# actionml/universal-recommender

Hardware: NVIDIA H100
Metric: CCO train events/sec to indicator model (higher is better)
Workload: dtype int32+f64

## Files before the change

universal_recommender_b200/csrc/cco_api.cu:

```cuda
#include <cuda_runtime.h>
#include <dlfcn.h>
#include <stdarg.h>
#include <stdio.h>
#include <stdlib.h>
#include <string.h>

#include <algorithm>
#include <charconv>
#include <cmath>
#include <functional>
#include <cub/cub.cuh>
#include <nvtx3/nvToolsExt.h>
#include <condition_variable>
#include <mutex>
#include <string>
#include <thread>
#include <unordered_map>
#include <vector>

#include "../../include/cco_b200.h"
#include "cco_kernels.cuh"
#include "cco_sampler.cuh"
#include "cco_format.cuh"
#include "cco_strings.cuh"
#include "cco_json.cuh"
#include "cco_events.cuh"
#include "cco_queries.cuh"
#include "cco_results.cuh"
#include "cco_index_pages.cuh"
#include "cco_index_write.cuh"
#include "cco_refresh.cuh"
#include "cco_intern.cuh"

namespace cco {

static thread_local char g_err[512] = "";
static int set_error(int code, const char *fmt, ...) {
  va_list ap;
  va_start(ap, fmt);
  vsnprintf(g_err, sizeof g_err, fmt, ap);
  va_end(ap);
  return code;
}
#define CK(expr)                                                                                      \
  do {                                                                                                \
    cudaError_t _e = (expr);                                                                          \
    if (_e != cudaSuccess)                                                                            \
      return set_error(_e == cudaErrorMemoryAllocation ? CCO_E_OOM : CCO_E_CUDA, "%s: %s (%s:%d)", #expr, \
                       cudaGetErrorString(_e), __FILE__, __LINE__);                                   \
  } while (0)
#define CKR(expr)            \
  do {                       \
    int _r = (expr);         \
    if (_r != CCO_OK) return _r; \
  } while (0)

typedef struct ncclComm *ncclComm_t;
typedef struct { char internal[128]; } ncclUniqueId;
struct Nccl {
  void *h = nullptr;
  int (*GetUniqueId)(ncclUniqueId *) = nullptr;
  int (*CommInitRank)(ncclComm_t *, int, ncclUniqueId, int) = nullptr;
  int (*CommInitAll)(ncclComm_t *, int, const int *) = nullptr;
  int (*CommDestroy)(ncclComm_t) = nullptr;
  int (*AllReduce)(const void *, void *, size_t, int, int, ncclComm_t, cudaStream_t) = nullptr;
  int (*AllGather)(const void *, void *, size_t, int, ncclComm_t, cudaStream_t) = nullptr;
  int (*Broadcast)(const void *, void *, size_t, int, int, ncclComm_t, cudaStream_t) = nullptr;
  int (*GroupStart)() = nullptr;
  int (*GroupEnd)() = nullptr;
  const char *(*GetErrorString)(int) = nullptr;
};
static Nccl g_nccl;
static std::mutex g_nccl_mu;
static int load_nccl() {
  std::lock_guard<std::mutex> lk(g_nccl_mu);
  if (g_nccl.h) return CCO_OK;
  void *h = dlopen("libnccl.so.2", RTLD_NOW | RTLD_GLOBAL);
  if (!h) h = dlopen("libnccl.so", RTLD_NOW | RTLD_GLOBAL);
  if (!h) return set_error(CCO_E_NCCL, "cannot load libnccl.so.2: %s", dlerror());
#define SYM(field, name)                                                         \
  *(void **)(&g_nccl.field) = dlsym(h, name);                                    \
  if (!g_nccl.field) return set_error(CCO_E_NCCL, "libnccl: missing symbol %s", name);
  SYM(GetUniqueId, "ncclGetUniqueId")
  SYM(CommInitRank, "ncclCommInitRank")
  SYM(CommInitAll, "ncclCommInitAll")
  SYM(CommDestroy, "ncclCommDestroy")
  SYM(AllReduce, "ncclAllReduce")
  SYM(AllGather, "ncclAllGather")
  SYM(Broadcast, "ncclBroadcast")
  SYM(GroupStart, "ncclGroupStart")
  SYM(GroupEnd, "ncclGroupEnd")
  SYM(GetErrorString, "ncclGetErrorString")
#undef SYM
  g_nccl.h = h;
  return CCO_OK;
}
constexpr int kNcclInt32 = 2, kNcclUint32 = 3, kNcclSum = 0, kNcclMax = 2;

}

using namespace cco;

struct PinnedBuf {
  void *p;
  size_t cap;
  bool used;
};

struct GroupShared {
  int world = 0;
  std::mutex mu;
  std::condition_variable cv;
  int arrived = 0;
  unsigned long long generation = 0;
  std::vector<long long> totals;
  struct cco_result *merged = nullptr;
  int status = 0;
  char err[512] = "";
  void barrier() {
    std::unique_lock<std::mutex> lk(mu);
    const unsigned long long g = generation;
    if (++arrived == world) {
      arrived = 0;
      ++generation;
      cv.notify_all();
    } else {
      cv.wait(lk, [&] { return generation != g; });
    }
  }
};

struct cco_ctx {
  int device = 0, rank = 0, world = 1;
  int sm_count = 0;
  size_t smem_optin = 0;
  cudaStream_t stream = nullptr, copy_stream = nullptr;
  cudaEvent_t ev[8] = {};
  cudaEvent_t tev[2] = {};
  cudaEvent_t copy_ev[2] = {};
  cudaStream_t bin_stream[8] = {};
  cudaStream_t sched_stream = nullptr;
  cudaEvent_t bin_ev[9] = {};
  std::vector<PinnedBuf> pinned;
  std::mutex mu;
  ncclComm_t comm = nullptr;
  int launches = 0;
  int32_t key_range_cap = 0;
  uint64_t intern_mask = ~0ULL;
  unsigned char *mail_h = nullptr, *mail_d = nullptr;
  size_t mail_used = 0;
  struct MailItem { void *dst; size_t off, n; int group; };
  std::vector<MailItem> mail_pending;
  std::vector<cudaEvent_t> mail_ev;
  int mail_group = 0;
  unsigned char *arena = nullptr;
  size_t arena_bytes = 0, arena_used = 0;
  int arena_live = 0;
  bool arena_registered = false;
  struct Slab { unsigned char *p; size_t cap; };
  std::vector<Slab> slabs;
  size_t slab_idx = 0, slab_off = 0;
  bool slab_busy = false;
  std::vector<cudaEvent_t> ev_timing, ev_plain;
  size_t ev_timing_used = 0, ev_plain_used = 0;
  std::vector<cco_ctx *> members;
  GroupShared *gshared = nullptr;

  void *pinned_get(size_t bytes, bool for_result = true) {
    std::lock_guard<std::mutex> lk(mu);
    if (bytes == 0) bytes = 16;
    if (arena && for_result) {
      const size_t off = (arena_used + 255) & ~(size_t)255;
      if (off + bytes <= arena_bytes) {
        arena_used = off + bytes;
        ++arena_live;
        return arena + off;
      }
    }
    int best = -1;
    for (size_t i = 0; i < pinned.size(); ++i)
      if (!pinned[i].used && pinned[i].cap >= bytes && (best < 0 || pinned[i].cap < pinned[best].cap)) best = (int)i;
    if (best >= 0) {
      pinned[best].used = true;
      return pinned[best].p;
    }
    void *p = nullptr;
    size_t cap = (bytes + (1u << 20) - 1) & ~((size_t)(1u << 20) - 1);
    if (cudaHostAlloc(&p, cap, cudaHostAllocPortable) != cudaSuccess) return nullptr;
    pinned.push_back({p, cap, true});
    return p;
  }
  void pinned_put(void *p) {
    std::lock_guard<std::mutex> lk(mu);
    if (arena && (unsigned char *)p >= arena && (unsigned char *)p < arena + arena_bytes) {
      if (--arena_live <= 0) { arena_live = 0; arena_used = 0; }
      return;
    }
    for (auto &b : pinned)
      if (b.p == p) b.used = false;
  }
};

struct ResultMat {
  int64_t row_begin = 0, row_end = 0;
  int32_t n_cols = 0;
  int64_t *row_ptr = nullptr;
  int32_t *col = nullptr;
  double *llr = nullptr;
  int32_t *cnt = nullptr;
  int32_t key_ranges = 1;
};
struct cco_dataset {
  cco_ctx *ctx = nullptr;
  int n_mats = 0;
  long long n_users = 0;
  long long row_base = 0, n_local = 0;
  std::vector<long long> n_cols, nnz;
  std::vector<long long *> rp;
  std::vector<int32_t *> col;
  std::vector<void *> rp_alloc, col_alloc;
  std::vector<long long> q_lo, q_hi;
  std::vector<cudaEvent_t> ready;
  bool h2d_pending = false;
  bool validated = false;
  bool whole = false;
  float ms_h2d = 0;
  std::vector<cco_dictionary_t> dicts;
};

struct cco_result {
  cco_ctx *ctx = nullptr;
  std::vector<ResultMat> mats;
  cco_stats_t stats;
};

namespace cco {

struct Arena {
  cudaStream_t s;
  cco_ctx *c;
  std::vector<void *> ptrs;
  std::vector<size_t> sizes;
  static constexpr size_t kSlabMax = 8u << 20, kSlabBytes = 64u << 20;
  explicit Arena(cudaStream_t st, cco_ctx *ctx = nullptr) : s(st), c(ctx && !ctx->slab_busy ? ctx : nullptr) {
    if (c) {
      c->slab_busy = true;
      c->slab_idx = 0;
      c->slab_off = 0;
    }
  }
  ~Arena() {
    for (void *p : ptrs) cudaFreeAsync(p, s);
    if (c) c->slab_busy = false;
  }
  void *bump(size_t bytes) {
    bytes = (bytes + 255) & ~(size_t)255;
    while (true) {
      if (c->slab_idx < c->slabs.size()) {
        cco_ctx::Slab &sl = c->slabs[c->slab_idx];
        if (c->slab_off + bytes <= sl.cap) {
          void *p = sl.p + c->slab_off;
          c->slab_off += bytes;
          return p;
        }
        ++c->slab_idx;
        c->slab_off = 0;
        continue;
      }
      void *p = nullptr;
      if (cudaMalloc(&p, kSlabBytes) != cudaSuccess) return nullptr;
      c->slabs.push_back({(unsigned char *)p, kSlabBytes});
    }
  }
  template <typename T>
  int alloc(T **out, size_t n) {
    void *p = nullptr;
    size_t bytes = std::max<size_t>(n * sizeof(T), 16);
    if (c && bytes <= kSlabMax) {
      p = bump(bytes);
      if (!p) return set_error(CCO_E_OOM, "cudaMalloc(scratch slab) failed");
      *out = (T *)p;
      return CCO_OK;
    }
    cudaError_t e = cudaMallocAsync(&p, bytes, s);
    if (e != cudaSuccess) return set_error(CCO_E_OOM, "cudaMallocAsync(%zu bytes): %s", bytes, cudaGetErrorString(e));
    ptrs.push_back(p);
    sizes.push_back(bytes);
    *out = (T *)p;
    return CCO_OK;
  }
  size_t take(void *p) {
    for (size_t i = 0; i < ptrs.size(); ++i)
      if (ptrs[i] == p) {
        const size_t b = sizes[i];
        ptrs.erase(ptrs.begin() + i);
        sizes.erase(sizes.begin() + i);
        return b;
      }
    return 0;
  }
  void release(void *p) {
    for (size_t i = 0; i < ptrs.size(); ++i)
      if (ptrs[i] == p) {
        cudaFreeAsync(p, s);
        ptrs.erase(ptrs.begin() + i);
        sizes.erase(sizes.begin() + i);
        return;
      }
  }
};
static int pooled_event(cco_ctx *c, bool timing, cudaEvent_t *out) {
  std::vector<cudaEvent_t> &pool = timing ? c->ev_timing : c->ev_plain;
  size_t &used = timing ? c->ev_timing_used : c->ev_plain_used;
  if (used == pool.size()) {
    cudaEvent_t e;
    CK(timing ? cudaEventCreate(&e) : cudaEventCreateWithFlags(&e, cudaEventDisableTiming));
    pool.push_back(e);
  }
  *out = pool[used++];
  return CCO_OK;
}

static inline void nvtx_push(const char *name) { nvtxRangePushA(name); }
static inline void nvtx_pop() { nvtxRangePop(); }
struct NvtxRange {
  explicit NvtxRange(const char *name) { nvtx_push(name); }
  ~NvtxRange() { nvtx_pop(); }
};

static inline int grid_for(long long work_items, int block, int sm_count, int waves = 8) {
  long long g = (work_items + block - 1) / block;
  long long cap = (long long)sm_count * waves;
  if (g > cap) g = cap;
  if (g < 1) g = 1;
  return (int)g;
}

constexpr size_t kMailBytes = 1 << 16;
static int mail_fetch(cco_ctx *c, void *dst_host, const void *src_dev, size_t n) {
  size_t off = (c->mail_used + 7) & ~(size_t)7;
  if (off + n > kMailBytes) return set_error(CCO_E_CUDA, "internal: mailbox overflow");
  k_mail_bytes<<<1, 128, 0, c->stream>>>(c->mail_d + off, (const unsigned char *)src_dev, (int)n);
  c->mail_pending.push_back({dst_host, off, n, c->mail_group});
  c->mail_used = off + n;
  return CCO_OK;
}
static int mail_close(cco_ctx *c, int *group) {
  const int g = c->mail_group;
  while ((int)c->mail_ev.size() <= g) {
    cudaEvent_t e;
    CK(cudaEventCreateWithFlags(&e, cudaEventDisableTiming));
    c->mail_ev.push_back(e);
  }
  CK(cudaEventRecord(c->mail_ev[g], c->stream));
  c->mail_group = g + 1;
  if (group) *group = g;
  return CCO_OK;
}
static int mail_wait_group(cco_ctx *c, int g) {
  CK(cudaEventSynchronize(c->mail_ev[g]));
  CK(cudaGetLastError());
  for (auto &m : c->mail_pending)
    if (m.group == g) memcpy(m.dst, c->mail_h + m.off, m.n);
  return CCO_OK;
}
static void mail_reset(cco_ctx *c) {
  c->mail_pending.clear();
  c->mail_used = 0;
  c->mail_group = 0;
}
static int mail_wait(cco_ctx *c) {
  int g = 0;
  CKR(mail_close(c, &g));
  return mail_wait_group(c, g);
}

struct DevRaw {
  long long n_rows = 0;
  long long row_base = 0;
  int32_t n_cols = 0;
  long long nnz = 0;
  long long q_base = 0;
  long long *rp = nullptr;
  int32_t *col = nullptr;
};
struct DevMat {
  long long n_rows = 0;
  int32_t n_cols = 0;
  uint32_t *rp = nullptr;
  int32_t *col = nullptr;
  int32_t *marg = nullptr;
};

template <typename T>
static int exclusive_sum(cco_ctx *c, Arena &ar, const T *in, T *out, long long n, cudaStream_t on = nullptr) {
  if (!on) on = c->stream;
  size_t tb = 0;
  CK(cub::DeviceScan::ExclusiveSum(nullptr, tb, in, out, n, on));
  void *tmp;
  CKR(ar.alloc((char **)&tmp, tb));
  CK(cub::DeviceScan::ExclusiveSum(tmp, tb, in, out, n, on));
  ar.release(tmp);
  return CCO_OK;
}
template <typename K, typename V>
static int sort_pairs(cco_ctx *c, Arena &ar, long long n, K **k, V **v, int bits) {
  cudaStream_t s = c->stream;
  K *k1;
  V *v1;
  CKR(ar.alloc(&k1, std::max<long long>(n, 1)));
  CKR(ar.alloc(&v1, std::max<long long>(n, 1)));
  cub::DoubleBuffer<K> kb(*k, k1);
  cub::DoubleBuffer<V> vb(*v, v1);
  size_t tbytes = 0;
  CK(cub::DeviceRadixSort::SortPairs(nullptr, tbytes, kb, vb, n, 0, bits, s));
  void *tmp;
  CKR(ar.alloc((char **)&tmp, tbytes));
  CK(cub::DeviceRadixSort::SortPairs(tmp, tbytes, kb, vb, n, 0, bits, s));
  c->launches++;
  ar.release(tmp);
  ar.release(kb.Alternate());
  ar.release(vb.Alternate());
  *k = kb.Current();
  *v = vb.Current();
  return CCO_OK;
}
static int bits_for(long long n) {
  int b = 1;
  while ((1LL << b) < n) ++b;
  return b;
}

static int keys_to_csr(cco_ctx *c, Arena &ar, unsigned long long *k0, unsigned long long *k1, long long n, int bits, long long n_valid,
                       long long n_rows, int32_t *col, long long *rp, long long *n_unique) {
  cudaStream_t s = c->stream;
  cub::DoubleBuffer<unsigned long long> db(k0, k1);
  size_t tb = 0;
  CK(cub::DeviceRadixSort::SortKeys(nullptr, tb, db, n, 0, bits, s));
  void *tmp;
  CKR(ar.alloc((char **)&tmp, tb));
  CK(cub::DeviceRadixSort::SortKeys(tmp, tb, db, n, 0, bits, s));
  ar.release(tmp);
  unsigned long long *sorted = db.Current(), *other = db.Alternate();
  uint32_t *flag, *pos;
  CKR(ar.alloc(&flag, n_valid + 1));
  CKR(ar.alloc(&pos, n_valid + 1));
  CK(cudaMemsetAsync(flag + n_valid, 0, 4, s));
  k_unique_flags<<<grid_for(n_valid, 256, c->sm_count), 256, 0, s>>>(n_valid, sorted, flag);
  CKR(exclusive_sum(c, ar, flag, pos, n_valid + 1));
  uint32_t nuq = 0;
  CKR(mail_fetch(c, &nuq, pos + n_valid, 4));
  k_unique_scatter<<<grid_for(n_valid, 256, c->sm_count), 256, 0, s>>>(n_valid, sorted, flag, pos, other, col);
  CKR(mail_wait(c));
  k_rowptr_from_keys<<<grid_for(n_rows + 1, 256, c->sm_count), 256, 0, s>>>(n_rows, nuq, other, rp);
  c->launches += 3;
  ar.release(flag);
  ar.release(pos);
  *n_unique = nuq;
  return CCO_OK;
}

static int canonicalize_device(cco_ctx *c, Arena &ar, DevRaw &m) {
  if (m.nnz == 0) return CCO_OK;
  unsigned long long *k0, *k1;
  CKR(ar.alloc(&k0, m.nnz));
  CKR(ar.alloc(&k1, m.nnz));
  k_expand_keys<<<grid_for(m.n_rows * kSG, 256, c->sm_count), 256, 0, c->stream>>>(m.n_rows, m.rp, m.col, k0);
  c->launches++;
  long long n_unique = 0;
  CKR(keys_to_csr(c, ar, k0, k1, m.nnz, 32 + bits_for(m.n_rows), m.nnz, m.n_rows, m.col + m.q_base, m.rp, &n_unique));
  m.col += m.q_base;
  m.q_base = 0;
  m.nnz = n_unique;
  CK(cudaGetLastError());
  ar.release(k0);
  ar.release(k1);
  return CCO_OK;
}

struct HeavyRows {
  int32_t *list = nullptr;
  int *n = nullptr;
};
static int list_heavy_rows(cco_ctx *c, Arena &ar, const DevRaw &raw, HeavyRows *h) {
  CKR(ar.alloc(&h->list, std::max<long long>(raw.n_rows, 1)));
  CKR(ar.alloc(&h->n, 1));
  CK(cudaMemsetAsync(h->n, 0, 4, c->stream));
  if (raw.n_rows > 0) {
    k_list_heavy_rows<<<grid_for(raw.n_rows, 256, c->sm_count), 256, 0, c->stream>>>(raw.n_rows, raw.rp, h->list, h->n);
    c->launches++;
  }
  return CCO_OK;
}
static void launch_check(cco_ctx *c, const DevRaw &raw, const HeavyRows &h, int *flags) {
  if (raw.n_rows <= 0) return;
  const long long q_lo = raw.q_base, q_hi = raw.q_base + raw.nnz;
  k_check_rows<kSG><<<grid_for(raw.n_rows * kSG, 256, c->sm_count), 256, 0, c->stream>>>(raw.n_rows, raw.n_cols, raw.rp, raw.col, q_lo, q_hi,
                                                                                       nullptr, nullptr, flags);
  k_check_rows<32><<<c->sm_count * 4, 256, 0, c->stream>>>(raw.n_rows, raw.n_cols, raw.rp, raw.col, q_lo, q_hi, h.list, h.n, flags);
  c->launches += 2;
}
struct SampleScratch {
  unsigned long long *col_thr = nullptr;
  uint8_t *keep = nullptr;
};
static int sample_scratch(cco_ctx *c, Arena &ar, const DevRaw &raw, const int32_t *raw_counts, int32_t m, SampleScratch *sc) {
  CKR(ar.alloc(&sc->col_thr, std::max<int32_t>(raw.n_cols, 1)));
  CKR(ar.alloc(&sc->keep, std::max<long long>(raw.nnz, 1)));
  if (raw.n_cols > 0) {
    k_col_thresholds<<<grid_for(raw.n_cols, 256, c->sm_count, 4), 256, 0, c->stream>>>(raw.n_cols, raw_counts, m, sc->col_thr);
    c->launches++;
  }
  return CCO_OK;
}
static void launch_count(cco_ctx *c, const DevRaw &raw, const SampleScratch &sc, int32_t m, int32_t seed, uint32_t flags, const int *bad,
                         uint32_t *kept, int32_t *new_counts) {
  if (raw.n_rows <= 0 || raw.nnz <= 0) return;
  const long long q_lo = raw.q_base, q_hi = raw.q_base + raw.nnz;
  const long long n_chunks = (raw.nnz + kSampleChunk - 1) / kSampleChunk;
  k_sample_count<<<grid_for(n_chunks * 32, 256, c->sm_count), 256, 0, c->stream>>>(raw.n_rows, raw.row_base, raw.rp, raw.col, raw.n_cols, q_lo, q_hi,
                                                                                  sc.col_thr, m, seed, flags, bad, kept, new_counts, sc.keep);
  c->launches++;
}
static int launch_write(cco_ctx *c, Arena &ar, const DevRaw &raw, const SampleScratch &sc, int32_t *dst) {
  if (raw.n_rows <= 0 || raw.nnz <= 0) return CCO_OK;
  long long *n_sel;
  CKR(ar.alloc(&n_sel, 1));
  size_t tb = 0;
  CK(cub::DeviceSelect::Flagged(nullptr, tb, raw.col + raw.q_base, sc.keep, dst, n_sel, (long long)raw.nnz, c->stream));
  void *tmp;
  CKR(ar.alloc((char **)&tmp, tb));
  CK(cub::DeviceSelect::Flagged(tmp, tb, raw.col + raw.q_base, sc.keep, dst, n_sel, (long long)raw.nnz, c->stream));
  ar.release(tmp);
  c->launches += 2;
  return CCO_OK;
}

constexpr int kHistCopies = 16;
static bool hist_fits_smem(const cco_ctx *c, int32_t n_cols) { return ((size_t)n_cols + 1) / 2 * 4 <= c->smem_optin; }
static int count_raw_columns(cco_ctx *c, Arena &ar, const std::vector<DevRaw> &raw, const std::vector<long long> &col_off, const cudaEvent_t *ready,
                             int *verdict, int32_t **counts_out) {
  cudaStream_t s = c->stream;
  const int n_mats = (int)raw.size();
  const long long total_cols = col_off[n_mats];
  const long long copy_stride = std::max<long long>(total_cols, 1);
  bool copies = false;
  for (int i = 0; i < n_mats; ++i) copies = copies || (raw[i].n_rows > 0 && !hist_fits_smem(c, raw[i].n_cols));
  const int n_copies = copies ? kHistCopies : 1;
  int32_t *counts;
  CKR(ar.alloc(&counts, (size_t)copy_stride * n_copies));
  CK(cudaMemsetAsync(counts, 0, sizeof(int32_t) * (size_t)copy_stride * n_copies, s));
  *counts_out = counts;
  std::vector<int> fit;
  for (int i = 0; i < n_mats; ++i)
    if (raw[i].n_rows > 0 && hist_fits_smem(c, raw[i].n_cols)) fit.push_back(i);
  for (size_t b0 = 0; b0 < fit.size(); b0 += kHistSegs) {
    const size_t b1 = std::min(fit.size(), b0 + kHistSegs);
    HistBatch hb{};
    long long nnz_sum = 0;
    int32_t max_cols = 0;
    for (size_t t = b0; t < b1; ++t) {
      nnz_sum += raw[fit[t]].nnz;
      max_cols = std::max(max_cols, raw[fit[t]].n_cols);
    }
    const size_t smem = ((size_t)max_cols + 1) / 2 * 4;
    const int per_sm = std::max(1, std::min<int>(2048 / kHistThreads, (int)(c->smem_optin / std::max<size_t>(smem + 1024, 1))));
    const long long target = (long long)c->sm_count * per_sm;
    for (size_t t = b0; t < b1; ++t) {
      const int i = fit[t];
      if (ready) CK(cudaStreamWaitEvent(s, ready[i], 0));
      const long long share = nnz_sum > 0 ? (target * raw[i].nnz + nnz_sum - 1) / nnz_sum : 1;
      const long long need = (raw[i].nnz + kHistMinEntries - 1) / kHistMinEntries;
      HistSeg &g = hb.seg[hb.n++];
      g.col = raw[i].col + raw[i].q_base;
      g.rp = raw[i].rp;
      g.nnz = raw[i].nnz;
      g.n_rows = raw[i].n_rows;
      g.q_lo = raw[i].q_base;
      g.q_hi = raw[i].q_base + raw[i].nnz;
      g.counts = counts + col_off[i];
      g.verdict = verdict ? verdict + 2 * i : nullptr;
      g.n_cols = raw[i].n_cols;
      g.cta0 = hb.cta_end;
      hb.cta_end += (int32_t)std::max(1LL, std::min(share, need));
    }
    CK(cudaFuncSetAttribute(k_col_counts_smem, cudaFuncAttributeMaxDynamicSharedMemorySize, (int)smem));
    k_col_counts_smem<<<hb.cta_end, kHistThreads, smem, s>>>(hb);
    c->launches++;
  }
  for (int i = 0; i < n_mats && copies; ++i) {
    if (raw[i].n_rows == 0 || hist_fits_smem(c, raw[i].n_cols)) continue;
    if (ready) CK(cudaStreamWaitEvent(s, ready[i], 0));
    int *v = verdict ? verdict + 2 * i : nullptr;
    if (v) {
      k_check_row_ptr<<<grid_for(raw[i].n_rows, 256, c->sm_count), 256, 0, s>>>(raw[i].n_rows, raw[i].rp, raw[i].q_base, raw[i].q_base + raw[i].nnz, v);
      c->launches++;
    }
    if (raw[i].nnz > 0) {
      k_col_histogram_flat<true><<<grid_for(raw[i].nnz, 256, c->sm_count), 256, 0, s>>>(raw[i].nnz, raw[i].col + raw[i].q_base, raw[i].n_cols,
                                                                                       counts + col_off[i], kHistCopies, copy_stride, v);
      c->launches++;
    }
  }
  if (copies) {
    k_sum_copies<<<grid_for(total_cols, 256, c->sm_count), 256, 0, s>>>(total_cols, kHistCopies, copy_stride, counts);
    c->launches++;
  }
  if (ready)
    for (int i = 0; i < n_mats; ++i) CK(cudaStreamWaitEvent(s, ready[i], 0));
  return CCO_OK;
}

static int nccl_check(int rc, const char *what) {
  if (rc != 0) return set_error(CCO_E_NCCL, "%s: %s", what, g_nccl.GetErrorString(rc));
  return CCO_OK;
}

static int downsample_all(cco_ctx *c, Arena &ar, const std::vector<DevRaw> &raw, const int *d_check , long long U,
                          const int32_t *raw_counts, int32_t *marg_all, const std::vector<long long> &col_off,
                          const cco_indicator_params_t *params, int32_t seed, uint32_t flags, std::vector<DevMat> &dm,
                          const cudaEvent_t *stage_ev ) {
  cudaStream_t s = c->stream;
  const int W = c->world, r = c->rank, n_mats = (int)raw.size();
  const long long S = (U + W - 1) / W;
  std::vector<uint32_t *> kept(n_mats, nullptr);
  std::vector<SampleScratch> sc(n_mats);
  for (int i = 0; i < n_mats; ++i) {
    DevMat *out = &dm[i];
    out->n_rows = U;
    out->n_cols = raw[i].n_cols;
    out->marg = marg_all + col_off[i];
    CKR(ar.alloc(&kept[i], (size_t)(W * S + 1)));
    CKR(ar.alloc(&out->rp, U + 1));
    CK(cudaMemsetAsync(kept[i], 0, sizeof(uint32_t) * (size_t)(W * S + 1), s));
    CKR(sample_scratch(c, ar, raw[i], raw_counts + col_off[i], params[i].max_interactions, &sc[i]));
    launch_count(c, raw[i], sc[i], params[i].max_interactions, seed, flags, d_check + 2 * i, kept[i], out->marg);
  }
  CK(cudaEventRecord(stage_ev[0], s));
  if (W > 1) {
    if (S > 0) {
      g_nccl.GroupStart();
      for (int i = 0; i < n_mats; ++i) {
        int rc = g_nccl.AllGather(kept[i] + (size_t)r * S, kept[i], (size_t)S, kNcclUint32, c->comm, s);
        if (rc != 0) { g_nccl.GroupEnd(); return nccl_check(rc, "ncclAllGather(kept counts)"); }
      }
      CKR(nccl_check(g_nccl.GroupEnd(), "ncclGroupEnd(kept counts)"));
    }
    if (col_off[n_mats] > 0)
      CKR(nccl_check(g_nccl.AllReduce(marg_all, marg_all, (size_t)col_off[n_mats], kNcclInt32, kNcclSum, c->comm, s), "ncclAllReduce(marginals)"));
  }
  std::vector<uint32_t> edge((size_t)n_mats * (W + 1), 0);
  for (int i = 0; i < n_mats; ++i) {
    CKR(exclusive_sum(c, ar, kept[i], dm[i].rp, U + 1));
    ar.release(kept[i]);
    if (W > 1)
      for (int q = 0; q <= W; ++q) CKR(mail_fetch(c, &edge[(size_t)i * (W + 1) + q], dm[i].rp + std::min<long long>((long long)q * S, U), 4));
  }
  CK(cudaEventRecord(stage_ev[1], s));
  if (W > 1) CKR(mail_wait(c));
  std::vector<long long> cap(n_mats, 0);
  std::vector<int32_t *> gathered(n_mats, nullptr);
  for (int i = 0; i < n_mats; ++i) {
    if (W == 1) {
      CKR(ar.alloc(&dm[i].col, std::max<long long>(raw[i].nnz, 1)));
      CKR(launch_write(c, ar, raw[i], sc[i], dm[i].col));
    } else {
      for (int q = 0; q < W; ++q) cap[i] = std::max<long long>(cap[i], (long long)edge[(size_t)i * (W + 1) + q + 1] - edge[(size_t)i * (W + 1) + q]);
      CKR(ar.alloc(&dm[i].col, std::max<long long>(edge[(size_t)i * (W + 1) + W], 1)));
      if (cap[i] > 0) {
        CKR(ar.alloc(&gathered[i], (size_t)(cap[i] * W)));
        CKR(launch_write(c, ar, raw[i], sc[i], gathered[i] + (size_t)r * cap[i]));
      }
    }
    ar.release(sc[i].col_thr);
    ar.release(sc[i].keep);
  }
  CK(cudaEventRecord(stage_ev[2], s));
  if (W > 1) {
    g_nccl.GroupStart();
    for (int i = 0; i < n_mats; ++i) {
      if (!gathered[i]) continue;
      int rc = g_nccl.AllGather(gathered[i] + (size_t)r * cap[i], gathered[i], (size_t)cap[i], kNcclInt32, c->comm, s);
      if (rc != 0) { g_nccl.GroupEnd(); return nccl_check(rc, "ncclAllGather(column blocks)"); }
    }
    CKR(nccl_check(g_nccl.GroupEnd(), "ncclGroupEnd(column blocks)"));
    for (int i = 0; i < n_mats; ++i) {
      if (!gathered[i]) continue;
      dim3 grid((unsigned)std::max(1, std::min(c->sm_count * 8 / W, 1024)), (unsigned)W);
      k_pack_blocks<<<grid, 256, 0, s>>>(W, S, U, cap[i], dm[i].rp, gathered[i], dm[i].col);
      c->launches++;
      ar.release(gathered[i]);
    }
  }
  CK(cudaEventRecord(stage_ev[3], s));
  CK(cudaGetLastError());
  return CCO_OK;
}


struct BinCfg {
  int group;
  int slots;
  int cap;
  int cbuf;
  int caux, keep_max, final_max;
  bool dense;
  bool bitmap;
  bool sorted;
  int bm_words;
  size_t region;
  size_t smem;
  int ctas_per_sm;
};

static int next_pow2(int x) {
  int p = 1;
  while (p < x) p <<= 1;
  return p;
}

template <int GROUP>
static int launch_rows_t(cco_ctx *c, const RowArgs &a, BinCfg &cfg, cudaStream_t st) {
  constexpr int CTA = GROUP == 32 ? 64 : GROUP;
  int occ = 1;
  void (*kern)(const RowArgs) = cfg.dense ? k_rows<GROUP, true> : k_rows<GROUP, false>;
  if constexpr (GROUP == 512 || GROUP == 256)
    if (cfg.bitmap) kern = k_rows<GROUP, false, true>;
  if constexpr (GROUP == 32)
    if (cfg.sorted) kern = k_rows<32, false, false, true>;
  CK(cudaFuncSetAttribute(kern, cudaFuncAttributeMaxDynamicSharedMemorySize, (int)cfg.smem));
  CK(cudaOccupancyMaxActiveBlocksPerMultiprocessor(&occ, kern, CTA, cfg.smem));
  kern<<<c->sm_count * std::max(occ, 1) * 4, CTA, cfg.smem, st>>>(a);
  cfg.ctas_per_sm = occ;
  c->launches++;
  CK(cudaGetLastError());
  return CCO_OK;
}
static int launch_rows(cco_ctx *c, const RowArgs &a, BinCfg &cfg, cudaStream_t st) {
  switch (cfg.group) {
    case 1024: return launch_rows_t<1024>(c, a, cfg, st);
    case 512: return launch_rows_t<512>(c, a, cfg, st);
    case 256: return launch_rows_t<256>(c, a, cfg, st);
    case 128: return launch_rows_t<128>(c, a, cfg, st);
    case 32: return launch_rows_t<32>(c, a, cfg, st);
  }
  return set_error(CCO_E_INVALID_ARG, "internal: bad bin config");
}

static BinCfg make_cfg(cco_ctx *c, int group, int want_slots, int top_k, int n_cols_b) {
  BinCfg f;
  const int groups = group == 32 ? 2 : 1;
  f.group = group;
  f.final_max = next_pow2(top_k);
  f.cbuf = next_pow2(top_k + std::max(group, 128) + (group == 32 ? 64 : 0));
  if (group == 32 && top_k + 32 <= 96) f.cbuf = 128;
  f.keep_max = std::max(f.final_max, (f.cbuf - group) / 2);
  f.caux = group == 32 ? 0 : f.keep_max;
  size_t fixed = (size_t)(f.cbuf + f.caux) * 16 + 2 * 256 + 512 + 1024 + (size_t)(group / 32) * 256;
  size_t avail = (c->smem_optin - 1024) / groups;
  int max_slots = (int)((avail - fixed) / 4) & ~1023;
  f.slots = std::min(want_slots, max_slots);
  f.cap = f.slots / 2;
  f.dense = n_cols_b <= f.slots;
  f.bitmap = false;
  f.sorted = false;
  f.bm_words = 0;
  f.region = (fixed + (size_t)f.slots * 4 + 15) & ~(size_t)15;
  f.smem = f.region * groups;
  f.ctas_per_sm = 1;
  return f;
}

static bool use_bitmap(BinCfg &f, uint32_t max_w, int top_k, int n_cols_b) {
  if (f.dense || (f.group != 512 && f.group != 256)) return false;
  const long long seg = 32LL * (f.group / 32);
  const long long rep = (std::max<long long>(max_w, 64) + seg - 1) / seg * seg;
  const long long bm = ((long long)n_cols_b + 31) / 32;
  if (rep + bm + top_k > f.slots) return false;
  f.bitmap = true;
  f.slots = (int)rep;
  f.bm_words = (int)bm;
  return true;
}

static bool use_sorted(BinCfg &f, uint32_t max_w, int count_bits) {
  constexpr int kAliased = 256 + 64;
  if (f.dense || f.group != 32 || max_w > 1024u) return false;
  const int slots = std::max(2 * (int)max_w - kAliased, (int)max_w);
  const int kb = 32 - count_bits, passes = (kb + 8) / 9;
  const int dbits = std::max((kb + passes - 1) / passes, 6);
  if (slots > f.slots || (long long)passes << (dbits - 1) > 4LL * f.cbuf) return false;
  f.sorted = true;
  f.region -= (size_t)(f.slots - slots) * 4;
  f.smem = f.region * 2;
  f.slots = slots;
  return true;
}

static double llr_error_bound(long long n_users) {
  const double n = (double)n_users;
  return n > 1.0 ? std::ldexp(n * std::log(n), -47) : 0.0;
}
static bool cut_exact(long long n_users, int32_t max_marg_a, int32_t max_marg_b) {
  const double n = (double)n_users, r = (double)max_marg_a, c = (double)max_marg_b;
  if (r <= 0.0 || c <= 0.0) return true;
  double g = 2.0 / std::min(r * c, 0.5 * n);
  const double d = n - c - r + 1.0;
  if (d > 0.0) g = std::max(g, 2.0 * (1.0 / c - (r - 1.0) / d));
  return g > 2.0 * llr_error_bound(n_users);
}

struct BinPlan {
  std::vector<BinCfg> cfgs;
  int32_t *d_bounds = nullptr;
};
static bool packed_bits(long long n_keys, long long k11_max, int *key_bits, int *count_bits) {
  int kb = 1;
  while (((1LL << kb) - 1) <= n_keys) ++kb;
  *key_bits = kb;
  *count_bits = 32 - kb;
  return *count_bits >= 1 && k11_max < (1LL << *count_bits);
}
static int plan_bins(cco_ctx *c, Arena &ar, int32_t n_items_a, int32_t n_cols_b, int count_bits, int32_t max_marg_a,
                     int32_t max_marg_b, long long n_users, int k_eff, bool emit_all, const uint32_t *sorted_work, cudaStream_t ss,
                     BinPlan *bp) {
  const bool warp_ok = k_eff + 32 <= 256;
  struct BinSpec { int group, slots; uint32_t max_w; };
  std::vector<BinSpec> spec = {{1024, 1 << 20, 0xffffffffu}, {1024, 1 << 20, 0xffffffffu}, {512, 16384, 8192u}, {256, 8192, 4096u}};
  if (warp_ok) {
    spec.push_back({128, 4096, 2048u});
    spec.push_back({32, 2048, 1024u});
    spec.push_back({32, 1024, 512u});
    spec.push_back({32, 512, 256u});
  } else {
    spec.push_back({128, 4096, 2048u});
  }
  const int kBins = (int)spec.size();
  std::vector<BinCfg> &cfgs = bp->cfgs;
  cfgs.resize(kBins);
  for (int b = 0; b < kBins; ++b) cfgs[b] = make_cfg(c, spec[b].group, spec[b].slots, k_eff, n_cols_b);
  std::vector<uint32_t> h_thr(kBins);
  for (int b = 0; b < kBins; ++b) {
    const BinCfg &f = cfgs[std::min(b + 1, kBins - 1)];
    uint32_t lim = b + 1 < kBins ? spec[b + 1].max_w : 0u;
    if (b + 1 < kBins && !f.dense) lim = std::min<uint32_t>(lim, (uint32_t)f.cap);
    h_thr[b] = lim;
    if (b > 0) h_thr[b] = std::min(h_thr[b], h_thr[b - 1]);
  }
  const bool bitmap_ok = !emit_all && cut_exact(n_users, max_marg_a, max_marg_b) &&
                         2ull * (unsigned long long)std::max(max_marg_a, 0) * (unsigned long long)std::max(max_marg_b, 0) <
                             (unsigned long long)n_users;
  for (int b = 1; b < kBins && bitmap_ok; ++b) {
    use_bitmap(cfgs[b], h_thr[b - 1], k_eff, n_cols_b);
    use_sorted(cfgs[b], h_thr[b - 1], count_bits);
  }
  if (!bp->d_bounds) CKR(ar.alloc(&bp->d_bounds, kBins + 3));
  BinThresholds bt;
  memset(&bt, 0, sizeof bt);
  for (int b = 0; b < kBins; ++b) bt.t[b] = h_thr[b];
  k_bin_bounds<<<1, 32, 0, ss>>>(n_items_a, sorted_work, kBins, bt, bp->d_bounds);
  c->launches++;
  return CCO_OK;
}
static int launch_bins(cco_ctx *c, const RowArgs &a, BinPlan &bp, cudaStream_t s) {
  std::vector<BinCfg> &cfgs = bp.cfgs;
  CK(cudaEventRecord(c->bin_ev[8], s));
  for (int b = 0; b < (int)cfgs.size(); ++b) {
    if (b == 0 && cfgs[1].dense) continue;
    RowArgs ab = a;
    ab.bin_bounds = bp.d_bounds;
    ab.bin = b;
    ab.slots = cfgs[b].slots;
    ab.cap = cfgs[b].cap;
    ab.tsize_x16 = 32;
    ab.cbuf = cfgs[b].cbuf;
    ab.caux = cfgs[b].caux;
    ab.keep_max = cfgs[b].keep_max;
    ab.final_max = cfgs[b].final_max;
    ab.group_smem_bytes = (int32_t)cfgs[b].region;
    ab.bm_words = cfgs[b].bm_words;
    CK(cudaStreamWaitEvent(c->bin_stream[b], c->bin_ev[8], 0));
    CKR(launch_rows(c, ab, cfgs[b], c->bin_stream[b]));
    CK(cudaEventRecord(c->bin_ev[b], c->bin_stream[b]));
    CK(cudaStreamWaitEvent(s, c->bin_ev[b], 0));
  }
  return CCO_OK;
}

static int key_shift_for(int32_t n_cols_b) {
  int sh = 0;
  while (((long long)std::max(n_cols_b - 1, 0) >> sh) >= kCutBins) ++sh;
  return sh;
}

struct KeyRange { int32_t k0, k1, max_marg; };
static bool plan_key_ranges(const int32_t *first_key_of_cb, int32_t max_marg_b, int32_t n_keys, int32_t max_marg_a,
                            int32_t max_keys, std::vector<KeyRange> *plan) {
  const int32_t *fk_end = first_key_of_cb + (size_t)max_marg_b + 2;
  auto marg = [&](int32_t k) { return (int32_t)(std::upper_bound(first_key_of_cb, fk_end, k) - first_key_of_cb) - 1; };
  auto fits = [&](int32_t k0, int32_t k1) {
    int kb, cb;
    return packed_bits((long long)k1 - k0, std::min<long long>(max_marg_a, marg(k1 - 1)), &kb, &cb);
  };
  plan->clear();
  for (int32_t k0 = 0; k0 < n_keys;) {
    const int32_t top = max_keys > 0 ? (int32_t)std::min<long long>(n_keys, (long long)k0 + max_keys) : n_keys;
    if (!fits(k0, k0 + 1)) return false;
    int32_t lo = k0 + 1, hi = top;
    while (lo < hi) {
      const int32_t mid = lo + (hi - lo + 1) / 2;
      if (fits(k0, mid)) lo = mid; else hi = mid - 1;
    }
    plan->push_back({k0, lo, marg(lo - 1)});
    k0 = lo;
  }
  return true;
}

struct IndicatorState {
  int mail_group = -1;
  long long rec[7] = {0, 0, 0, 0, 0, 0, 0};
  cudaEvent_t packed = nullptr;
  long long *out_ptr = nullptr;
  int32_t *p_col = nullptr, *p_cnt = nullptr;
  double *p_llr = nullptr;
  int32_t n_items_a = 0, n_cols_b = 0;
  int n_ranges = 1;
  bool emit_all = false;
};

static int enqueue_indicator(cco_ctx *c, Arena &ar, const uint32_t *at_ptr, const int32_t *at_users, int32_t n_items_a,
                             const int32_t *marg_a, int32_t max_marg_a, int32_t max_marg_b, const DevMat &B, long long n_users,
                             bool self, const cco_indicator_params_t &prm, uint32_t flags, bool emit_all, cudaEvent_t inputs_ready,
                             cudaEvent_t ev_begin, cudaEvent_t ev_end, IndicatorState *st) {
  cudaStream_t s = c->stream;
  const int32_t n_cols_b = B.n_cols;
  const int rank = c->rank, world = c->world;
  st->n_items_a = n_items_a;
  st->n_cols_b = n_cols_b;
  st->emit_all = emit_all;
  uint32_t *row_work, *masked, *sorted_work;
  unsigned long long *work64;
  long long *work_prefix;
  int32_t *ids, *rows_sorted, *d_pb = nullptr;
  size_t sort_tb = 0, order_tb = 0;
  if (n_items_a > 0)
    CK(cub::DeviceRadixSort::SortPairsDescending(nullptr, sort_tb, (const uint32_t *)nullptr, (uint32_t *)nullptr, (const int32_t *)nullptr,
                                                 (int32_t *)nullptr, n_items_a, 0, 32, s));
  int cb_bits = 1;
  while ((1LL << cb_bits) <= (long long)max_marg_b) ++cb_bits;
  cub::DoubleBuffer<uint32_t> order_cb(nullptr, nullptr);
  cub::DoubleBuffer<int32_t> order_id(nullptr, nullptr);
  if (n_cols_b > 0) CK(cub::DeviceRadixSort::SortPairs(nullptr, order_tb, order_cb, order_id, n_cols_b, 0, cb_bits, s));
  const bool beside = inputs_ready && ar.c && ((size_t)n_items_a + 1) * 8 <= Arena::kSlabMax && sort_tb <= Arena::kSlabMax &&
                      (size_t)n_cols_b * 4 <= Arena::kSlabMax && order_tb <= Arena::kSlabMax &&
                      ((size_t)max_marg_b + 2) * 4 <= Arena::kSlabMax;
  cudaStream_t ss = beside ? c->sched_stream : s;
  if (beside) CK(cudaStreamWaitEvent(ss, inputs_ready, 0));
  CKR(ar.alloc(&row_work, n_items_a + 1));
  CKR(ar.alloc(&masked, n_items_a + 1));
  CKR(ar.alloc(&work64, n_items_a + 1));
  CKR(ar.alloc(&work_prefix, n_items_a + 1));
  CKR(ar.alloc(&ids, n_items_a + 1));
  CKR(ar.alloc(&sorted_work, n_items_a + 1));
  CKR(ar.alloc(&rows_sorted, n_items_a + 1));
  CK(cudaMemsetAsync(work64 + n_items_a, 0, 8, ss));
  k_row_work<<<grid_for((long long)n_items_a * kSG, 256, c->sm_count), 256, 0, ss>>>(n_items_a, at_ptr, at_users, B.rp,
                                                                                  row_work, work64, ids, nullptr);
  c->launches++;
  CKR(exclusive_sum(c, ar, (const long long *)work64, work_prefix, (long long)n_items_a + 1, ss));
  if (world > 1) {
    CKR(ar.alloc(&d_pb, world + 1));
    k_partition_rows<<<1, ((world + 1 + 31) / 32) * 32, 0, ss>>>(work_prefix, n_items_a, world, d_pb);
    c->launches++;
  }
  k_mask_work<<<grid_for(n_items_a, 256, c->sm_count), 256, 0, ss>>>(n_items_a, row_work, d_pb, rank, masked);
  c->launches++;
  if (n_items_a > 0) {
    void *tmp;
    CKR(ar.alloc((char **)&tmp, sort_tb));
    CK(cub::DeviceRadixSort::SortPairsDescending(tmp, sort_tb, masked, sorted_work, ids, rows_sorted, n_items_a, 0, 32, ss));
    ar.release(tmp);
  }
  const int k_eff = emit_all ? 1 : prm.top_k;
  int key_bits, count_bits;
  const long long k11_max = std::min<long long>(max_marg_a, max_marg_b);
  const bool fits = packed_bits(n_cols_b, k11_max, &key_bits, &count_bits);
  const bool split = n_cols_b > 0 && (c->key_range_cap > 0 || (!fits && (flags & CCO_FLAG_KEY_RANGES)));
  if (!fits && !split)
    return set_error(CCO_E_UNSUPPORTED,
                     "co-occurrence counts up to %lld over %d columns do not fit the packed 32-bit accumulator word "
                     "(key %d bits + count %d bits): lower maxItemsPerUser/maxEventsPerEventType for this event type, "
                     "or train it in key ranges with CCO_FLAG_KEY_RANGES (\"Limits\" in include/cco_b200.h)",
                     k11_max, n_cols_b, key_bits, count_bits);
  st->n_ranges = 1;
  BinPlan bins;
  if (!split)
    CKR(plan_bins(c, ar, n_items_a, n_cols_b, count_bits, max_marg_a, max_marg_b, n_users, k_eff, emit_all, sorted_work, ss, &bins));
  int32_t *key_of_col, *first_key_of_cb, *order_id0, *order_id1;
  uint32_t *order_cb0, *order_cb1;
  const int32_t n_order = std::max<int32_t>(n_cols_b, 1);
  CKR(ar.alloc(&key_of_col, n_order));
  CKR(ar.alloc(&first_key_of_cb, (size_t)max_marg_b + 2));
  CKR(ar.alloc(&order_cb0, n_order));
  CKR(ar.alloc(&order_cb1, n_order));
  CKR(ar.alloc(&order_id0, n_order));
  CKR(ar.alloc(&order_id1, n_order));
  order_cb = cub::DoubleBuffer<uint32_t>(order_cb0, order_cb1);
  order_id = cub::DoubleBuffer<int32_t>(order_id0, order_id1);
  if (n_cols_b > 0) {
    k_col_order_init<<<grid_for(n_cols_b, 256, c->sm_count, 4), 256, 0, ss>>>(n_cols_b, B.marg, order_cb0, order_id0);
    void *tmp;
    CKR(ar.alloc((char **)&tmp, order_tb));
    CK(cub::DeviceRadixSort::SortPairs(tmp, order_tb, order_cb, order_id, n_cols_b, 0, cb_bits, ss));
    ar.release(tmp);
    k_col_order<<<grid_for(n_cols_b, 256, c->sm_count, 4), 256, 0, ss>>>(n_cols_b, max_marg_b, order_cb.Current(), order_id.Current(),
                                                                        key_of_col, first_key_of_cb);
    k_relabel_cols<<<c->sm_count * 8, 256, 0, ss>>>(B.rp + B.n_rows, key_of_col, B.col);
    c->launches += 3;
  }
  const int32_t *marg_key = reinterpret_cast<const int32_t *>(order_cb.Current()), *col_of_key = order_id.Current();
  if (beside) {
    cudaEvent_t scheduled;
    CKR(pooled_event(c, false, &scheduled));
    CK(cudaEventRecord(scheduled, ss));
    CK(cudaStreamWaitEvent(s, scheduled, 0));
  }
  ColTerm *col_terms;
  CKR(ar.alloc(&col_terms, std::max<int32_t>(n_cols_b, 1)));
  if (n_cols_b > 0) {
    k_col_terms<<<grid_for(n_cols_b, 256, c->sm_count, 4), 256, 0, s>>>(n_cols_b, marg_key, col_of_key, n_users, flags, col_terms);
    c->launches++;
  }
  int32_t stride = emit_all ? n_cols_b : std::min<int32_t>(prm.top_k, n_cols_b);
  if (stride < 1) stride = 1;
  int32_t *o_col, *o_cnt, *o_len;
  double *o_llr = nullptr;
  unsigned long long *d_distinct;
  int *d_err;
  size_t cells = (size_t)std::max(n_items_a, 1) * stride;
  CKR(ar.alloc(&o_col, cells));
  CKR(ar.alloc(&o_cnt, cells));
  if (!emit_all) CKR(ar.alloc(&o_llr, cells));
  CKR(ar.alloc(&o_len, n_items_a + 1));
  CKR(ar.alloc(&d_distinct, 2));
  CKR(ar.alloc(&d_err, 1));
  CK(cudaMemsetAsync(o_len, 0, sizeof(int32_t) * ((size_t)n_items_a + 1), s));
  CK(cudaMemsetAsync(d_distinct, 0, 16, s));
  CK(cudaMemsetAsync(d_err, 0, 4, s));
  RowArgs a;
  memset(&a, 0, sizeof a);
  a.at_ptr = at_ptr;
  a.at_users = at_users;
  a.b_ptr = B.rp;
  a.b_col = B.col;
  a.marg_a = marg_a;
  a.marg_b = marg_key;
  a.key_of_col = key_of_col;
  a.first_key_of_cb = first_key_of_cb;
  a.key_shift = key_shift_for(n_cols_b);
  a.max_marg_b = max_marg_b;
  a.col_terms = col_terms;
  a.rows_sorted = rows_sorted;
  a.row_work = row_work;
  a.n_cols_b = n_cols_b;
  a.n_users = n_users;
  a.self = self ? 1 : 0;
  a.top_k = k_eff;
  a.has_min_llr = prm.has_min_llr;
  a.min_llr = prm.min_llr;
  a.cut_ok = cut_exact(n_users, max_marg_a, max_marg_b) ? 1 : 0;
  a.llr_eps2 = 2.0 * llr_error_bound(n_users);
  a.flags = flags;
  a.count_bits = count_bits;
  a.out_stride = stride;
  a.out_col = o_col;
  a.out_llr = o_llr;
  a.out_cnt = o_cnt;
  a.out_len = o_len;
  a.stat_distinct = d_distinct;
  a.stat_evaluated = d_distinct + 1;
  a.err_flag = d_err;
  a.emit_all = emit_all ? 1 : 0;
  a.key_base = 0;
  if (ev_begin) CK(cudaEventRecord(ev_begin, s));
  if (!split) {
    if (n_items_a > 0) CKR(launch_bins(c, a, bins, s));
  } else {
    const int32_t n_fk = max_marg_b + 2;
    int32_t *h_fk = (int32_t *)c->pinned_get(sizeof(int32_t) * ((size_t)n_fk + 1), false);
    if (!h_fk) return set_error(CCO_E_OOM, "pinned host allocation failed");
    struct PutBack { cco_ctx *c; void *p; ~PutBack() { c->pinned_put(p); } } put_back{c, h_fk};
    CK(cudaMemcpyAsync(h_fk, first_key_of_cb, sizeof(int32_t) * (size_t)n_fk, cudaMemcpyDeviceToHost, s));
    CK(cudaMemcpyAsync(h_fk + n_fk, B.rp + B.n_rows, sizeof(uint32_t), cudaMemcpyDeviceToHost, s));
    CK(cudaStreamSynchronize(s));
    std::vector<KeyRange> plan;
    if (!plan_key_ranges(h_fk, max_marg_b, n_cols_b, max_marg_a, c->key_range_cap, &plan))
      return set_error(CCO_E_UNSUPPORTED,
                       "co-occurrence counts up to %lld do not fit the packed 32-bit accumulator word even in a key range of one "
                       "column (at most 2^30 - 1): lower maxItemsPerUser/maxEventsPerEventType for this event type "
                       "(\"Limits\" in include/cco_b200.h)", k11_max);
    const long long nnz_b = (long long)(uint32_t)h_fk[n_fk], U = B.n_rows;
    st->n_ranges = (int)plan.size();
    uint32_t *r_cnt, *r_ptr;
    int32_t *r_col, *fk_r, *t_col = nullptr, *t_cnt = nullptr, *t_len = nullptr;
    double *t_llr = nullptr;
    void *scan_tmp, *sort_tmp;
    size_t scan_tb = 0;
    CKR(ar.alloc(&r_cnt, U + 1));
    CKR(ar.alloc(&r_ptr, U + 1));
    CK(cub::DeviceScan::ExclusiveSum(nullptr, scan_tb, r_cnt, r_ptr, U + 1, s));
    CKR(ar.alloc(&r_col, std::max<long long>(nnz_b, 1)));
    CKR(ar.alloc(&fk_r, (size_t)max_marg_b + 2));
    CKR(ar.alloc((char **)&scan_tmp, scan_tb));
    CKR(ar.alloc((char **)&sort_tmp, sort_tb));
    BinPlan bp;
    if (plan.size() > 1) {
      CKR(ar.alloc(&t_col, cells));
      CKR(ar.alloc(&t_cnt, cells));
      if (!emit_all) CKR(ar.alloc(&t_llr, cells));
      CKR(ar.alloc(&t_len, n_items_a + 1));
    }
    const int split_grid = grid_for(U * 32, 256, c->sm_count);
    for (size_t r = 0; r < plan.size(); ++r) {
      const KeyRange kr = plan[r];
      const int32_t n_r = kr.k1 - kr.k0;
      k_split_range<false><<<split_grid, 256, 0, s>>>(U, B.rp, B.col, kr.k0, kr.k1, r_cnt, nullptr);
      CK(cub::DeviceScan::ExclusiveSum(scan_tmp, scan_tb, r_cnt, r_ptr, U + 1, s));
      k_split_range<true><<<split_grid, 256, 0, s>>>(U, B.rp, B.col, kr.k0, kr.k1, r_ptr, r_col);
      c->launches += 2;
      k_row_work<<<grid_for((long long)n_items_a * kSG, 256, c->sm_count), 256, 0, s>>>(n_items_a, at_ptr, at_users, r_ptr, row_work,
                                                                                     work64, ids, nullptr);
      k_mask_work<<<grid_for(n_items_a, 256, c->sm_count), 256, 0, s>>>(n_items_a, row_work, d_pb, rank, masked);
      c->launches += 2;
      if (n_items_a > 0)
        CK(cub::DeviceRadixSort::SortPairsDescending(sort_tmp, sort_tb, masked, sorted_work, ids, rows_sorted, n_items_a, 0, 32, s));
      k_range_first_keys<<<grid_for((long long)kr.max_marg + 2, 256, c->sm_count), 256, 0, s>>>(kr.max_marg + 2, first_key_of_cb, kr.k0,
                                                                                             n_r, fk_r);
      c->launches++;
      int kb_r, cbits_r;
      packed_bits(n_r, std::min<long long>(max_marg_a, kr.max_marg), &kb_r, &cbits_r);
      CKR(plan_bins(c, ar, n_items_a, n_r, cbits_r, max_marg_a, kr.max_marg, n_users, k_eff, emit_all, sorted_work, s, &bp));
      RowArgs ar_r = a;
      ar_r.b_ptr = r_ptr;
      ar_r.b_col = r_col;
      ar_r.marg_b = marg_key + kr.k0;
      ar_r.col_terms = col_terms + kr.k0;
      ar_r.first_key_of_cb = fk_r;
      ar_r.key_base = kr.k0;
      ar_r.key_shift = key_shift_for(n_r);
      ar_r.max_marg_b = kr.max_marg;
      ar_r.n_cols_b = n_r;
      ar_r.cut_ok = cut_exact(n_users, max_marg_a, kr.max_marg) ? 1 : 0;
      ar_r.count_bits = cbits_r;
      if (r > 0) {
        ar_r.out_col = t_col;
        ar_r.out_llr = t_llr;
        ar_r.out_cnt = t_cnt;
        ar_r.out_len = t_len;
        CK(cudaMemsetAsync(t_len, 0, sizeof(int32_t) * ((size_t)n_items_a + 1), s));
      }
      if (n_items_a > 0) CKR(launch_bins(c, ar_r, bp, s));
      if (r > 0 && n_items_a > 0) {
        k_merge_range<<<grid_for((long long)n_items_a * 32, 256, c->sm_count), 256, 0, s>>>(n_items_a, stride, k_eff, emit_all ? 1 : 0, o_col,
                                                                                         o_llr, o_cnt, o_len, t_col, t_llr, t_cnt, t_len);
        c->launches++;
      }
    }
  }
  if (ev_end) CK(cudaEventRecord(ev_end, s));
  long long *len64, *rec_d;
  CKR(ar.alloc(&len64, n_items_a + 1));
  CKR(ar.alloc(&st->out_ptr, n_items_a + 1));
  CKR(ar.alloc(&rec_d, 8));
  k_len_to_i64<<<grid_for((long long)n_items_a + 1, 256, c->sm_count), 256, 0, s>>>(n_items_a, o_len, d_pb, rank, len64);
  c->launches++;
  CKR(exclusive_sum(c, ar, len64, st->out_ptr, (long long)n_items_a + 1));
  CKR(ar.alloc(&st->p_col, cells));
  if (!(flags & CCO_FLAG_RESULT_NO_COUNT) || emit_all) CKR(ar.alloc(&st->p_cnt, cells));
  if (!emit_all && !(flags & CCO_FLAG_RESULT_NO_LLR)) CKR(ar.alloc(&st->p_llr, cells));
  if (n_items_a > 0) {
    k_compact_rows<<<grid_for((long long)n_items_a * 32, 256, c->sm_count), 256, 0, s>>>(n_items_a, stride, st->out_ptr, o_col, o_llr,
                                                                                      o_cnt, st->p_col, st->p_llr, st->p_cnt);
    c->launches++;
  }
  k_indicator_record<<<1, 32, 0, s>>>(n_items_a, d_pb, rank, st->out_ptr, work_prefix, d_distinct, d_err, rec_d);
  c->launches++;
  CKR(mail_fetch(c, st->rec, rec_d, sizeof(long long) * 7));
  CKR(mail_close(c, &st->mail_group));
  if (!st->packed) CK(cudaEventCreateWithFlags(&st->packed, cudaEventDisableTiming));
  CK(cudaEventRecord(st->packed, s));
  CK(cudaGetLastError());
  for (void *p : {(void *)o_col, (void *)o_cnt, (void *)o_llr, (void *)len64})
    if (p) ar.release(p);
  return CCO_OK;
}

struct IndicatorOut {
  int64_t row_begin = 0, row_end = 0;
  int64_t nnz = 0;
  int64_t products = 0, distinct = 0, evaluated = 0;
};

static int finish_indicator(cco_ctx *c, IndicatorState *st, uint32_t flags, int index, ResultMat *rm, IndicatorOut *io) {
  CKR(mail_wait_group(c, st->mail_group));
  const int32_t lo = (int32_t)st->rec[0], hi = (int32_t)st->rec[1];
  const long long total = st->rec[2];
  io->row_begin = lo;
  io->row_end = hi;
  io->nnz = total;
  io->products = st->rec[3];
  io->distinct = st->rec[4];
  io->evaluated = st->rec[5];
  if (st->rec[6]) return set_error(CCO_E_CUDA, "internal: shared-memory hash table overflow");
  const int32_t n_my = hi - lo;
  cudaStream_t cs = c->copy_stream;
  CK(cudaStreamWaitEvent(cs, st->packed, 0));
  GroupShared *gs = c->gshared;
  int64_t *h_rp;
  int32_t *h_col, *h_cnt = nullptr;
  double *h_llr = nullptr;
  long long base = 0;
  if (gs) {
    {
      std::lock_guard<std::mutex> lk(gs->mu);
      gs->totals[c->rank] = total;
    }
    gs->barrier();
    long long grand = 0;
    for (int q = 0; q < gs->world; ++q) {
      if (q < c->rank) base += gs->totals[q];
      grand += gs->totals[q];
    }
    ResultMat &mm = gs->merged->mats[index];
    if (c->rank == 0) {
      cco_ctx *owner = gs->merged->ctx;
      mm.row_begin = 0;
      mm.row_end = st->n_items_a;
      mm.n_cols = st->n_cols_b;
      mm.row_ptr = (int64_t *)owner->pinned_get(sizeof(int64_t) * ((size_t)st->n_items_a + 1));
      mm.col = (int32_t *)owner->pinned_get(sizeof(int32_t) * (size_t)std::max<long long>(grand, 1));
      if (st->p_cnt) mm.cnt = (int32_t *)owner->pinned_get(sizeof(int32_t) * (size_t)std::max<long long>(grand, 1));
      if (st->p_llr) mm.llr = (double *)owner->pinned_get(sizeof(double) * (size_t)std::max<long long>(grand, 1));
      mm.key_ranges = st->n_ranges;
    }
    gs->barrier();
    if (!mm.row_ptr || !mm.col || (st->p_cnt && !mm.cnt) || (st->p_llr && !mm.llr)) return set_error(CCO_E_OOM, "pinned host allocation failed");
    h_rp = mm.row_ptr + lo;
    h_col = mm.col + base;
    h_cnt = mm.cnt ? mm.cnt + base : nullptr;
    h_llr = mm.llr ? mm.llr + base : nullptr;
    if (base != 0 && n_my >= 0) {
      k_add_i64<<<grid_for((long long)n_my + 1, 256, c->sm_count, 2), 256, 0, cs>>>((long long)n_my + 1, base, st->out_ptr + lo);
      c->launches++;
    }
    rm->row_begin = lo;
    rm->row_end = hi;
    rm->n_cols = st->n_cols_b;
    rm->key_ranges = st->n_ranges;
  } else {
    rm->row_begin = lo;
    rm->row_end = hi;
    rm->n_cols = st->n_cols_b;
    rm->key_ranges = st->n_ranges;
    rm->row_ptr = (int64_t *)c->pinned_get(sizeof(int64_t) * ((size_t)n_my + 1));
    rm->col = (int32_t *)c->pinned_get(sizeof(int32_t) * (size_t)std::max<long long>(total, 1));
    if (st->p_cnt) rm->cnt = (int32_t *)c->pinned_get(sizeof(int32_t) * (size_t)std::max<long long>(total, 1));
    if (st->p_llr) rm->llr = (double *)c->pinned_get(sizeof(double) * (size_t)std::max<long long>(total, 1));
    if (!rm->row_ptr || !rm->col || (st->p_cnt && !rm->cnt) || (st->p_llr && !rm->llr))
      return set_error(CCO_E_OOM, "pinned host allocation failed");
    h_rp = rm->row_ptr;
    h_col = rm->col;
    h_cnt = rm->cnt;
    h_llr = rm->llr;
  }
  CK(cudaMemcpyAsync(h_rp, st->out_ptr + lo, sizeof(int64_t) * ((size_t)n_my + 1), cudaMemcpyDeviceToHost, cs));
  if (total > 0 && !(flags & CCO_FLAG_RESULT_ON_DEVICE)) {
    CK(cudaMemcpyAsync(h_col, st->p_col, sizeof(int32_t) * (size_t)total, cudaMemcpyDeviceToHost, cs));
    if (h_cnt) CK(cudaMemcpyAsync(h_cnt, st->p_cnt, sizeof(int32_t) * (size_t)total, cudaMemcpyDeviceToHost, cs));
    if (h_llr) CK(cudaMemcpyAsync(h_llr, st->p_llr, sizeof(double) * (size_t)total, cudaMemcpyDeviceToHost, cs));
  }
  return CCO_OK;
}

static int validate_host(int32_t n_mats, const cco_csr_t *mats, const cco_indicator_params_t *params) {
  if (n_mats < 1 || !mats || !params) return set_error(CCO_E_INVALID_ARG, "need at least the primary matrix and its params");
  for (int i = 0; i < n_mats; ++i) {
    const cco_csr_t &m = mats[i];
    if (!m.row_ptr) return set_error(CCO_E_INVALID_ARG, "matrix %d: null row_ptr", i);
    if (m.n_rows < 0 || m.n_rows >= 0x7fffffffLL) return set_error(CCO_E_INVALID_ARG, "matrix %d: n_rows out of range", i);
    if (m.n_cols < 0 || m.n_cols >= 0x7ffffffe) return set_error(CCO_E_INVALID_ARG, "matrix %d: n_cols out of range", i);
    if (m.n_rows != mats[0].n_rows)
      return set_error(CCO_E_SHAPE_MISMATCH, "matrix %d has %lld rows, the primary has %lld: all event types share the user dictionary",
                       i, (long long)m.n_rows, (long long)mats[0].n_rows);
    if (m.row_ptr[0] != 0) return set_error(CCO_E_INVALID_ARG, "matrix %d: row_ptr[0] != 0", i);
    long long nnz = m.row_ptr[m.n_rows];
    if (nnz < 0 || nnz >= 0xffffffffLL) return set_error(CCO_E_UNSUPPORTED, "matrix %d: nnz %lld outside [0, 2^32)", i, nnz);
    if (nnz > 0 && !m.col_idx) return set_error(CCO_E_INVALID_ARG, "matrix %d: null col_idx", i);
    if (params[i].max_interactions < 1) return set_error(CCO_E_INVALID_ARG, "matrix %d: max_interactions must be >= 1", i);
    if (params[i].top_k < 1) return set_error(CCO_E_INVALID_ARG, "matrix %d: top_k must be >= 1", i);
    if (params[i].top_k > CCO_MAX_TOP_K)
      return set_error(CCO_E_UNSUPPORTED, "matrix %d: top_k %d > CCO_MAX_TOP_K (%d)", i, params[i].top_k, CCO_MAX_TOP_K);
    if (params[i].has_min_llr && params[i].min_llr != params[i].min_llr)
      return set_error(CCO_E_INVALID_ARG, "matrix %d: min_llr is NaN", i);
  }
  return CCO_OK;
}

static inline void user_block(long long U, int W, int r, long long *lo, long long *hi) {
  const long long S = (U + W - 1) / W;
  *lo = std::min<long long>((long long)r * S, U);
  *hi = std::min<long long>(*lo + S, U);
}

static void dataset_release(cco_dataset *d) {
  if (!d) return;
  cudaSetDevice(d->ctx->device);
  for (auto p : d->rp_alloc)
    if (p) cudaFreeAsync(p, d->ctx->stream);
  for (auto p : d->col_alloc)
    if (p) cudaFreeAsync(p, d->ctx->stream);
  for (auto e : d->ready)
    if (e) cudaEventDestroy(e);
  for (auto &dc : d->dicts) {
    if (dc.offsets) d->ctx->pinned_put((void *)dc.offsets);
    if (dc.bytes) d->ctx->pinned_put((void *)dc.bytes);
  }
  delete d;
}

static DevRaw block_of(const cco_dataset *d, int i) {
  DevRaw r;
  r.n_rows = d->n_local;
  r.row_base = d->row_base;
  r.n_cols = (int32_t)d->n_cols[i];
  r.q_base = d->q_lo[i];
  r.nnz = d->q_hi[i] - d->q_lo[i];
  r.rp = d->rp[i];
  r.col = d->col[i];
  return r;
}

static int dataset_validate(cco_ctx *c, cco_dataset *d, bool canonicalise) {
  cudaStream_t s = c->stream;
  const int n_mats = d->n_mats;
  mail_reset(c);
  Arena ar(s);
  int *d_flags;
  CKR(ar.alloc(&d_flags, 2 * n_mats));
  CK(cudaMemsetAsync(d_flags, 0, sizeof(int) * 2 * n_mats, s));
  for (int i = 0; i < n_mats; ++i) {
    CK(cudaStreamWaitEvent(s, d->ready[i], 0));
    if (d->n_local == 0) continue;
    const DevRaw r = block_of(d, i);
    HeavyRows hv;
    CKR(list_heavy_rows(c, ar, r, &hv));
    launch_check(c, r, hv, d_flags + 2 * i);
  }
  if (c->world > 1)
    CKR(nccl_check(g_nccl.AllReduce(d_flags, d_flags, (size_t)(2 * n_mats), kNcclInt32, kNcclMax, c->comm, s), "ncclAllReduce(check flags)"));
  std::vector<int> h(2 * n_mats);
  CK(cudaMemcpyAsync(h.data(), d_flags, sizeof(int) * 2 * n_mats, cudaMemcpyDeviceToHost, s));
  CK(cudaStreamSynchronize(s));
  CK(cudaGetLastError());
  for (int i = 0; i < n_mats; ++i)
    if (h[2 * i]) return set_error(CCO_E_INVALID_ARG, "matrix %d: row_ptr not monotone or column index out of [0, n_cols)", i);
  if (canonicalise)
    for (int i = 0; i < n_mats; ++i)
      if (h[2 * i + 1] && d->n_local > 0) {
        DevRaw r = block_of(d, i);
        CKR(canonicalize_device(c, ar, r));
        d->col[i] = r.col;
        d->q_lo[i] = 0;
        d->q_hi[i] = r.nnz;
        if (c->world == 1) d->nnz[i] = r.nnz;
      }
  CK(cudaStreamSynchronize(s));
  d->validated = canonicalise;
  return CCO_OK;
}

static int dataset_upload(cco_ctx *c, int32_t n_mats, const cco_csr_t *mats, uint32_t flags, cco_dataset **out, bool async = false) {
  CK(cudaSetDevice(c->device));
  cudaStream_t s = c->stream;
  cco_dataset *d = new cco_dataset();
  d->ctx = c;
  d->n_mats = n_mats;
  d->n_users = mats[0].n_rows;
  long long u_lo, u_hi;
  user_block(d->n_users, c->world, c->rank, &u_lo, &u_hi);
  d->row_base = u_lo;
  d->n_local = u_hi - u_lo;
  d->whole = c->world == 1;
  d->rp.assign(n_mats, nullptr);
  d->col.assign(n_mats, nullptr);
  d->rp_alloc.assign(n_mats, nullptr);
  d->col_alloc.assign(n_mats, nullptr);
  d->n_cols.assign(n_mats, 0);
  d->nnz.assign(n_mats, 0);
  d->q_lo.assign(n_mats, 0);
  d->q_hi.assign(n_mats, 0);
  d->ready.assign(n_mats, nullptr);
  struct G {
    cco_dataset *d;
    bool ok = false;
    ~G() {
      if (!ok) dataset_release(d);
    }
  } g{d};
  cudaStream_t cs = c->copy_stream;
  for (int i = 0; i < n_mats; ++i) {
    const cco_csr_t &m = mats[i];
    d->n_cols[i] = m.n_cols;
    d->nnz[i] = m.row_ptr[m.n_rows];
    const long long q0 = m.row_ptr[u_lo], q1 = m.row_ptr[u_hi];
    d->q_lo[i] = q0;
    d->q_hi[i] = q1;
    void *p = nullptr;
    cudaError_t e = cudaMallocAsync(&p, sizeof(int64_t) * ((size_t)d->n_local + 1), s);
    if (e != cudaSuccess) return set_error(CCO_E_OOM, "cudaMallocAsync row_ptr: %s", cudaGetErrorString(e));
    d->rp_alloc[i] = p;
    d->rp[i] = (long long *)p;
    e = cudaMallocAsync(&p, sizeof(int32_t) * (size_t)std::max<long long>(q1 - q0, 4), s);
    if (e != cudaSuccess) return set_error(CCO_E_OOM, "cudaMallocAsync col_idx: %s", cudaGetErrorString(e));
    d->col_alloc[i] = p;
    d->col[i] = (int32_t *)p - q0;
    CK(cudaEventCreateWithFlags(&d->ready[i], cudaEventDisableTiming));
  }
  CK(cudaEventRecord(c->copy_ev[0], s));
  CK(cudaStreamWaitEvent(cs, c->copy_ev[0], 0));
  CK(cudaEventRecord(c->ev[6], cs));
  for (int i = 0; i < n_mats; ++i) {
    const cco_csr_t &m = mats[i];
    const long long q0 = m.row_ptr[u_lo], q1 = m.row_ptr[u_hi];
    CK(cudaMemcpyAsync(d->rp_alloc[i], m.row_ptr + u_lo, sizeof(int64_t) * ((size_t)d->n_local + 1), cudaMemcpyHostToDevice, cs));
    if (q1 > q0)
      CK(cudaMemcpyAsync(d->col_alloc[i], m.col_idx + q0, sizeof(int32_t) * (size_t)(q1 - q0), cudaMemcpyHostToDevice, cs));
    CK(cudaEventRecord(d->ready[i], cs));
  }
  CK(cudaEventRecord(c->ev[7], cs));
  if (async && (flags & CCO_FLAG_ASSUME_CANONICAL)) {
    d->h2d_pending = true;
    g.ok = true;
    *out = d;
    return CCO_OK;
  }
  CKR(dataset_validate(c, d, !(flags & CCO_FLAG_ASSUME_CANONICAL)));
  CK(cudaEventElapsedTime(&d->ms_h2d, c->ev[6], c->ev[7]));
  g.ok = true;
  *out = d;
  return CCO_OK;
}

struct Prepared {
  std::vector<DevMat> dm;
  uint32_t *at_ptr = nullptr;
  int32_t *at_users = nullptr;
  int32_t *raw_counts = nullptr;
  std::vector<int32_t> max_marg;
  std::vector<uint32_t> nnz;
  cudaEvent_t stage[7] = {};
};
static int prepare(cco_ctx *c, Arena &ar, const cco_dataset *ds, const cco_indicator_params_t *params, int32_t seed, uint32_t flags,
                   Prepared *p) {
  cudaStream_t s = c->stream;
  const int n_mats = ds->n_mats;
  const long long n_users = ds->n_users;
  std::vector<DevRaw> raw(n_mats);
  for (int i = 0; i < n_mats; ++i) raw[i] = block_of(ds, i);
  for (auto &e : p->stage) CKR(pooled_event(c, true, &e));
  auto mark = [&](int k) { return cudaEventRecord(p->stage[k], s); };
  CK(cudaEventRecord(c->ev[1], s));
  nvtx_push("cco:prepare");
  long long total_cols = 0;
  std::vector<long long> col_off(n_mats + 1, 0);
  for (int i = 0; i < n_mats; ++i) {
    col_off[i] = total_cols;
    total_cols += raw[i].n_cols;
  }
  col_off[n_mats] = total_cols;
  const long long copy_stride = std::max<long long>(total_cols, 1);
  int32_t *marg_all;
  int *d_check;
  CKR(ar.alloc(&marg_all, (size_t)copy_stride));
  CKR(ar.alloc(&d_check, 2 * n_mats));
  CK(cudaMemsetAsync(marg_all, 0, sizeof(int32_t) * (size_t)copy_stride, s));
  CK(cudaMemsetAsync(d_check, 0, sizeof(int) * 2 * n_mats, s));
  CKR(count_raw_columns(c, ar, raw, col_off, ds->ready.data(), ds->validated ? nullptr : d_check, &p->raw_counts));
  CK(mark(0));
  if (c->world > 1) {
    if (total_cols > 0)
      CKR(nccl_check(g_nccl.AllReduce(p->raw_counts, p->raw_counts, (size_t)total_cols, kNcclInt32, kNcclSum, c->comm, s), "ncclAllReduce(raw counts)"));
    CKR(nccl_check(g_nccl.AllReduce(d_check, d_check, (size_t)(2 * n_mats), kNcclInt32, kNcclMax, c->comm, s), "ncclAllReduce(check flags)"));
  }
  CK(mark(1));
  std::vector<DevMat> &dm = p->dm;
  dm.assign(n_mats, DevMat());
  CKR(downsample_all(c, ar, raw, d_check, n_users, p->raw_counts, marg_all, col_off, params, seed, flags, dm, &p->stage[2]));
  const int32_t n_items_a = dm[0].n_cols;
  uint32_t *cursor;
  int32_t *d_max;
  CKR(ar.alloc(&p->at_ptr, n_items_a + 1));
  CKR(ar.alloc(&cursor, n_items_a + 1));
  CKR(ar.alloc(&d_max, n_mats));
  CKR(ar.alloc(&p->at_users, std::max<long long>(ds->nnz[0], 1)));
  CK(cudaMemsetAsync(d_max, 0, 4 * (size_t)n_mats, s));
  {
    uint32_t *marg_pad;
    CKR(ar.alloc(&marg_pad, n_items_a + 1));
    CK(cudaMemcpyAsync(marg_pad, dm[0].marg, sizeof(int32_t) * (size_t)n_items_a, cudaMemcpyDeviceToDevice, s));
    CK(cudaMemsetAsync(marg_pad + n_items_a, 0, 4, s));
    CKR(exclusive_sum(c, ar, marg_pad, p->at_ptr, (long long)n_items_a + 1));
    ar.release(marg_pad);
  }
  CK(cudaMemcpyAsync(cursor, p->at_ptr, sizeof(uint32_t) * ((size_t)n_items_a + 1), cudaMemcpyDeviceToDevice, s));
  k_transpose_entries<<<grid_for((ds->nnz[0] + kSampleChunk - 1) / kSampleChunk * 32, 256, c->sm_count), 256, 0, s>>>(n_users, dm[0].rp,
                                                                                                                     dm[0].col, cursor, p->at_users);
  c->launches++;
  for (int i = 0; i < n_mats; ++i)
    if (dm[i].n_cols > 0) {
      k_max_i32<<<grid_for(dm[i].n_cols, 256, c->sm_count, 2), 256, 0, s>>>(dm[i].n_cols, dm[i].marg, d_max + i);
      c->launches++;
    }
  p->max_marg.assign(n_mats, 0);
  p->nnz.assign(n_mats, 0);
  std::vector<int> h_check(2 * n_mats, 0);
  CKR(mail_fetch(c, p->max_marg.data(), d_max, 4 * (size_t)n_mats));
  CKR(mail_fetch(c, h_check.data(), d_check, sizeof(int) * 2 * (size_t)n_mats));
  for (int i = 0; i < n_mats; ++i) CKR(mail_fetch(c, &p->nnz[i], dm[i].rp + n_users, 4));
  CK(mark(6));
  CK(cudaEventRecord(c->ev[2], s));
  nvtx_pop();
  CKR(mail_wait(c));
  for (int i = 0; i < n_mats; ++i)
    if (h_check[2 * i]) return set_error(CCO_E_INVALID_ARG, "matrix %d: row_ptr not monotone or column index out of [0, n_cols)", i);
  return CCO_OK;
}

static int train_dataset(cco_ctx *c, const cco_dataset *ds, const cco_indicator_params_t *params, int32_t seed, uint32_t flags,
                         cco_result **out) {
  CK(cudaSetDevice(c->device));
  cudaStream_t s = c->stream;
  const int n_mats = ds->n_mats;
  mail_reset(c);
  c->ev_timing_used = c->ev_plain_used = 0;
  Arena ar(s, c);
  struct CopyJoin {
    cco_ctx *c;
    ~CopyJoin() {
      cudaStreamSynchronize(c->copy_stream);
      cudaStreamSynchronize(c->sched_stream);
    }
  } copy_join{c};
  cco_result *res = new cco_result();
  res->ctx = c;
  res->mats.resize(n_mats);
  memset(&res->stats, 0, sizeof res->stats);
  struct Guard {
    cco_result *r;
    bool ok = false;
    ~Guard() {
      if (!ok) cco_result_free(r);
    }
  } guard{res};
  std::vector<IndicatorState> ist(n_mats);
  for (auto &x : ist) CKR(pooled_event(c, false, &x.packed));
  cco_stats_t &st = res->stats;
  st.n_mats = n_mats;
  st.n_users = ds->n_users;
  st.ms_h2d = ds->ms_h2d;
  const bool h2d_pending = ds->h2d_pending;
  const long long n_users = ds->n_users;
  for (int i = 0; i < n_mats; ++i) st.nnz_in_total += ds->nnz[i];
  Prepared p;
  CKR(prepare(c, ar, ds, params, seed, flags, &p));
  for (int i = 0; i < n_mats && i < 16; ++i) st.nnz_downsampled[i] = p.nnz[i];

  const int32_t n_items_a = p.dm[0].n_cols;
  std::vector<IndicatorOut> io(n_mats);
  std::vector<cudaEvent_t> ev_rows(2 * n_mats, nullptr);
  for (auto &e : ev_rows) CKR(pooled_event(c, true, &e));
  for (int i = 0; i < n_mats; ++i) {
    nvtx_push("cco:indicator");
    CKR(enqueue_indicator(c, ar, p.at_ptr, p.at_users, n_items_a, p.dm[0].marg, p.max_marg[0], p.max_marg[i], p.dm[i], n_users, i == 0,
                          params[i], flags, false, c->ev[2], ev_rows[2 * i], ev_rows[2 * i + 1], &ist[i]));
    nvtx_pop();
    if (i > 0) CKR(finish_indicator(c, &ist[i - 1], flags, i - 1, &res->mats[i - 1], &io[i - 1]));
  }
  CKR(finish_indicator(c, &ist[n_mats - 1], flags, n_mats - 1, &res->mats[n_mats - 1], &io[n_mats - 1]));
  CK(cudaEventRecord(c->copy_ev[1], c->copy_stream));
  CK(cudaStreamWaitEvent(s, c->copy_ev[1], 0));
  CK(cudaEventRecord(c->ev[3], s));
  CK(cudaStreamSynchronize(s));
  CK(cudaStreamSynchronize(c->copy_stream));
  for (int i = 0; i < n_mats && i < 16; ++i) {
    st.products[i] = io[i].products;
    st.distinct_cells[i] = io[i].distinct;
    st.llr_evaluated[i] = io[i].evaluated;
    st.out_nnz[i] = io[i].nnz;
    CK(cudaEventElapsedTime(&st.ms_indicator[i], ev_rows[2 * i], ev_rows[2 * i + 1]));
  }
  if (h2d_pending) CK(cudaEventElapsedTime(&st.ms_h2d, c->ev[6], c->ev[7]));
  CK(cudaEventElapsedTime(&st.ms_prep_stage[0], c->ev[1], p.stage[0]));
  for (int k = 1; k <= 6; ++k) CK(cudaEventElapsedTime(&st.ms_prep_stage[k], p.stage[k - 1], p.stage[k]));
  CK(cudaEventElapsedTime(&st.ms_prepare, c->ev[1], c->ev[2]));
  CK(cudaEventElapsedTime(&st.ms_cooccurrence, c->ev[2], c->ev[3]));
  CK(cudaEventElapsedTime(&st.ms_total, c->ev[1], c->ev[3]));
  if (!h2d_pending) st.ms_total += st.ms_h2d;
  st.n_kernel_launches = c->launches;
  guard.ok = true;
  *out = res;
  return CCO_OK;
}

static int train_impl(cco_ctx *c, int32_t n_mats, const cco_csr_t *mats, const cco_indicator_params_t *params, int32_t seed,
                      uint32_t flags, cco_result **out) {
  c->launches = 0;
  cco_dataset *ds = nullptr;
  CKR(dataset_upload(c, n_mats, mats, flags, &ds, true));
  int rc = train_dataset(c, ds, params, seed, flags, out);
  cudaStreamSynchronize(c->copy_stream);
  dataset_release(ds);
  return rc;
}

static int train_group(cco_ctx *leader, int32_t n_mats, const cco_csr_t *mats, const cco_indicator_params_t *params, int32_t seed,
                       uint32_t flags, cco_result **out) {
  const int W = (int)leader->members.size();
  GroupShared *gs = leader->members[0]->gshared;
  cco_result *merged = new cco_result();
  merged->ctx = leader;
  merged->mats.resize(n_mats);
  memset(&merged->stats, 0, sizeof merged->stats);
  gs->merged = merged;
  gs->totals.assign(W, 0);
  gs->status = CCO_OK;
  gs->err[0] = 0;
  std::vector<cco_result *> part(W, nullptr);
  std::vector<std::thread> th;
  for (int r = 0; r < W; ++r)
    th.emplace_back([&, r]() {
      int rc = train_impl(leader->members[r], n_mats, mats, params, seed, flags, &part[r]);
      if (rc != CCO_OK) {
        std::lock_guard<std::mutex> lk(gs->mu);
        if (gs->status == CCO_OK) {
          gs->status = rc;
          snprintf(gs->err, sizeof gs->err, "GPU %d: %s", leader->members[r]->device, cco_last_error());
        }
      }
    });
  for (auto &t : th) t.join();
  gs->merged = nullptr;
  if (gs->status != CCO_OK) {
    for (auto p : part)
      if (p) cco_result_free(p);
    cco_result_free(merged);
    return set_error(gs->status, "%s", gs->err);
  }
  cco_stats_t &st = merged->stats;
  st = part[0]->stats;
  for (int r = 1; r < W; ++r) {
    const cco_stats_t &p = part[r]->stats;
    for (int i = 0; i < 16; ++i) {
      st.products[i] += p.products[i];
      st.distinct_cells[i] += p.distinct_cells[i];
      st.out_nnz[i] += p.out_nnz[i];
      st.llr_evaluated[i] += p.llr_evaluated[i];
      st.ms_indicator[i] = std::max(st.ms_indicator[i], p.ms_indicator[i]);
    }
    st.ms_h2d = std::max(st.ms_h2d, p.ms_h2d);
    st.ms_prepare = std::max(st.ms_prepare, p.ms_prepare);
    st.ms_cooccurrence = std::max(st.ms_cooccurrence, p.ms_cooccurrence);
    st.ms_total = std::max(st.ms_total, p.ms_total);
    st.n_kernel_launches += p.n_kernel_launches;
  }
  for (auto p : part) cco_result_free(p);
  *out = merged;
  return CCO_OK;
}

}

extern "C" {

int cco_abi_version(void) { return CCO_ABI_VERSION; }
const char *cco_last_error(void) { return g_err; }
const char *cco_status_string(int s) {
  switch (s) {
    case CCO_OK: return "ok";
    case CCO_E_INVALID_ARG: return "invalid argument";
    case CCO_E_CUDA: return "CUDA error";
    case CCO_E_NCCL: return "NCCL error";
    case CCO_E_OOM: return "out of memory";
    case CCO_E_SHAPE_MISMATCH: return "shape mismatch";
    case CCO_E_UNSUPPORTED: return "unsupported";
  }
  return "unknown";
}

int cco_device_count(void) {
  int n = 0;
  cudaError_t e = cudaGetDeviceCount(&n);
  if (e != cudaSuccess) return set_error(CCO_E_CUDA, "cudaGetDeviceCount: %s", cudaGetErrorString(e));
  int ok = 0;
  for (int i = 0; i < n; ++i) {
    cudaDeviceProp p;
    if (cudaGetDeviceProperties(&p, i) == cudaSuccess && p.major == 9 && p.minor == 0) ++ok;
  }
  return ok;
}

int cco_nccl_unique_id(unsigned char out[128]) {
  if (!out) return set_error(CCO_E_INVALID_ARG, "null output");
  CKR(load_nccl());
  ncclUniqueId id;
  int r = g_nccl.GetUniqueId(&id);
  if (r != 0) return set_error(CCO_E_NCCL, "ncclGetUniqueId: %s", g_nccl.GetErrorString(r));
  memcpy(out, id.internal, 128);
  return CCO_OK;
}

static int ctx_init_device(cco_ctx *c) {
  CK(cudaSetDevice(c->device));
  CK(cudaStreamCreateWithFlags(&c->stream, cudaStreamNonBlocking));
  CK(cudaStreamCreateWithFlags(&c->copy_stream, cudaStreamNonBlocking));
  for (auto &ev : c->ev) CK(cudaEventCreate(&ev));
  for (auto &ev : c->tev) CK(cudaEventCreate(&ev));
  for (auto &ev : c->copy_ev) CK(cudaEventCreateWithFlags(&ev, cudaEventDisableTiming));
  for (auto &st : c->bin_stream) CK(cudaStreamCreateWithFlags(&st, cudaStreamNonBlocking));
  int lo_pri = 0, hi_pri = 0;
  CK(cudaDeviceGetStreamPriorityRange(&lo_pri, &hi_pri));
  CK(cudaStreamCreateWithPriority(&c->sched_stream, cudaStreamNonBlocking, hi_pri));
  for (auto &ev : c->bin_ev) CK(cudaEventCreateWithFlags(&ev, cudaEventDisableTiming));
  CK(cudaHostAlloc((void **)&c->mail_h, kMailBytes, cudaHostAllocMapped | cudaHostAllocPortable));
  CK(cudaHostGetDevicePointer((void **)&c->mail_d, c->mail_h, 0));
  cudaMemPool_t pool;
  CK(cudaDeviceGetDefaultMemPool(&pool, c->device));
  uint64_t thr = UINT64_MAX;
  CK(cudaMemPoolSetAttribute(pool, cudaMemPoolAttrReleaseThreshold, &thr));
  return CCO_OK;
}

static int check_device(int device, cudaDeviceProp *p) {
  int n = 0;
  cudaError_t e = cudaGetDeviceCount(&n);
  if (e != cudaSuccess || n == 0)
    return set_error(CCO_E_CUDA, "no CUDA device (%s): this library has no CPU fallback",
                     e != cudaSuccess ? cudaGetErrorString(e) : "device count 0");
  if (device < 0 || device >= n) return set_error(CCO_E_INVALID_ARG, "device %d not in [0,%d)", device, n);
  CK(cudaGetDeviceProperties(p, device));
  if (p->major != 9 || p->minor != 0)
    return set_error(CCO_E_CUDA, "device %d is sm_%d%d; this build contains sm_90a code only", device, p->major, p->minor);
  return CCO_OK;
}

static int create_failed(cco_ctx *c, int st) {
  char keep[sizeof g_err];
  memcpy(keep, g_err, sizeof keep);
  cco_destroy(c);
  memcpy(g_err, keep, sizeof keep);
  return st;
}

int cco_create(const cco_config_t *cfg, cco_ctx_t **out) {
  if (!cfg || !out) return set_error(CCO_E_INVALID_ARG, "null argument");
  if (cfg->world_size < 1 || cfg->rank < 0 || cfg->rank >= cfg->world_size)
    return set_error(CCO_E_INVALID_ARG, "bad rank/world_size %d/%d", cfg->rank, cfg->world_size);
  if (cfg->world_size > 1023) return set_error(CCO_E_UNSUPPORTED, "world_size %d > 1023", cfg->world_size);
  cudaDeviceProp p;
  CKR(check_device(cfg->device, &p));
  if (cfg->world_size > 1 && !cfg->nccl_unique_id) return set_error(CCO_E_INVALID_ARG, "world_size > 1 needs nccl_unique_id");
  cco_ctx *c = new cco_ctx();
  c->device = cfg->device;
  c->rank = cfg->rank;
  c->world = cfg->world_size;
  c->sm_count = p.multiProcessorCount;
  c->smem_optin = p.sharedMemPerBlockOptin;
  auto init = [&]() -> int {
    CKR(ctx_init_device(c));
    if (cfg->result_arena && cfg->result_arena_bytes > 0) {
      CK(cudaHostRegister(cfg->result_arena, cfg->result_arena_bytes, cudaHostRegisterPortable));
      c->arena = (unsigned char *)cfg->result_arena;
      c->arena_bytes = cfg->result_arena_bytes;
      c->arena_registered = true;
    }
    if (c->world > 1) {
      CKR(load_nccl());
      ncclUniqueId id;
      memcpy(id.internal, cfg->nccl_unique_id, 128);
      int rc = g_nccl.CommInitRank(&c->comm, c->world, id, c->rank);
      if (rc != 0) return set_error(CCO_E_NCCL, "ncclCommInitRank: %s", g_nccl.GetErrorString(rc));
    }
    return CCO_OK;
  };
  const int st = init();
  if (st != CCO_OK) return create_failed(c, st);
  *out = c;
  return CCO_OK;
}

int cco_create_group(int32_t n_devices, const int32_t *devices, cco_ctx_t **out) {
  if (!devices || !out || n_devices < 1) return set_error(CCO_E_INVALID_ARG, "bad argument");
  if (n_devices > 1023) return set_error(CCO_E_UNSUPPORTED, "more than 1023 devices");
  std::vector<cudaDeviceProp> props(n_devices);
  for (int r = 0; r < n_devices; ++r) {
    CKR(check_device(devices[r], &props[r]));
    for (int q = 0; q < r; ++q)
      if (devices[q] == devices[r]) return set_error(CCO_E_INVALID_ARG, "device %d listed twice", devices[r]);
  }
  cco_ctx *leader = new cco_ctx();
  leader->device = devices[0];
  leader->world = 1;
  GroupShared *gs = new GroupShared();
  gs->world = n_devices;
  auto init = [&]() -> int {
    std::vector<ncclComm_t> comms(n_devices, nullptr);
    if (n_devices > 1) {
      CKR(load_nccl());
      std::vector<int> devs(devices, devices + n_devices);
      int rc = g_nccl.CommInitAll(comms.data(), n_devices, devs.data());
      if (rc != 0) return set_error(CCO_E_NCCL, "ncclCommInitAll: %s", g_nccl.GetErrorString(rc));
    }
    for (int r = 0; r < n_devices; ++r) {
      cco_ctx *m = new cco_ctx();
      m->device = devices[r];
      m->rank = r;
      m->world = n_devices;
      m->sm_count = props[r].multiProcessorCount;
      m->smem_optin = props[r].sharedMemPerBlockOptin;
      m->comm = comms[r];
      m->gshared = gs;
      leader->members.push_back(m);
      CKR(ctx_init_device(m));
    }
    CK(cudaSetDevice(devices[0]));
    return CCO_OK;
  };
  const int st = init();
  if (st != CCO_OK) {
    if (leader->members.empty()) delete gs;
    return create_failed(leader, st);
  }
  *out = leader;
  return CCO_OK;
}

int cco_destroy(cco_ctx_t *c) {
  if (!c) return CCO_OK;
  if (!c->members.empty()) {
    GroupShared *gs = c->members[0]->gshared;
    for (cco_ctx *m : c->members) {
      m->gshared = nullptr;
      cco_destroy(m);
    }
    c->members.clear();
    delete gs;
  }
  cudaSetDevice(c->device);
  if (c->stream) cudaStreamSynchronize(c->stream);
  if (c->copy_stream) cudaStreamSynchronize(c->copy_stream);
  if (c->comm) g_nccl.CommDestroy(c->comm);
  for (auto &b : c->pinned) cudaFreeHost(b.p);
  if (c->arena_registered) cudaHostUnregister(c->arena);
  if (c->mail_h) cudaFreeHost(c->mail_h);
  for (auto &ev : c->mail_ev) cudaEventDestroy(ev);
  for (auto &ev : c->ev_timing) cudaEventDestroy(ev);
  for (auto &ev : c->ev_plain) cudaEventDestroy(ev);
  for (auto &sl : c->slabs) cudaFree(sl.p);
  for (auto &ev : c->ev)
    if (ev) cudaEventDestroy(ev);
  for (auto &ev : c->tev)
    if (ev) cudaEventDestroy(ev);
  for (auto &ev : c->copy_ev)
    if (ev) cudaEventDestroy(ev);
  for (auto &st : c->bin_stream)
    if (st) cudaStreamDestroy(st);
  if (c->sched_stream) cudaStreamDestroy(c->sched_stream);
  for (auto &ev : c->bin_ev)
    if (ev) cudaEventDestroy(ev);
  if (c->stream) cudaStreamDestroy(c->stream);
  if (c->copy_stream) cudaStreamDestroy(c->copy_stream);
  delete c;
  return CCO_OK;
}

int cco_host_alloc(cco_ctx_t *c, size_t bytes, void **out) {
  if (!c || !out) return set_error(CCO_E_INVALID_ARG, "null argument");
  CK(cudaSetDevice(c->device));
  void *p = c->pinned_get(bytes, false);
  if (!p) return set_error(CCO_E_OOM, "cudaHostAlloc(%zu) failed", bytes);
  *out = p;
  return CCO_OK;
}
int cco_host_free(cco_ctx_t *c, void *p) {
  if (!c) return set_error(CCO_E_INVALID_ARG, "null context");
  if (p) c->pinned_put(p);
  return CCO_OK;
}

int cco_train(cco_ctx_t *ctx, int32_t n_mats, const cco_csr_t *mats, const cco_indicator_params_t *params, int32_t seed,
              uint32_t flags, cco_result_t **out) {
  if (!ctx || !out) return set_error(CCO_E_INVALID_ARG, "null argument");
  *out = nullptr;
  CKR(validate_host(n_mats, mats, params));
  if (!ctx->members.empty()) return train_group(ctx, n_mats, mats, params, seed, flags, out);
  return train_impl(ctx, n_mats, mats, params, seed, flags, out);
}

int cco_cooccurrences_idss(cco_ctx_t *ctx, int32_t n_mats, const cco_csr_t *mats, int32_t seed,
                           int32_t max_interesting_items_per_thing, int32_t max_num_interactions, uint32_t flags,
                           cco_result_t **out) {
  if (n_mats < 1) return set_error(CCO_E_INVALID_ARG, "need at least the primary matrix");
  std::vector<cco_indicator_params_t> p(n_mats);
  for (auto &q : p) {
    q.max_interactions = max_num_interactions;
    q.top_k = max_interesting_items_per_thing;
    q.has_min_llr = 0;
    q.min_llr = 0.0;
  }
  return cco_train(ctx, n_mats, mats, p.data(), seed, flags, out);
}

int cco_dataset_shape(const cco_dataset_t *ds, int32_t i, int64_t *n_rows, int32_t *n_cols, int64_t *nnz) {
  if (!ds || i < 0 || i >= ds->n_mats) return set_error(CCO_E_INVALID_ARG, "bad dataset/index");
  if (n_rows) *n_rows = ds->n_users;
  if (n_cols) *n_cols = (int32_t)ds->n_cols[i];
  if (nnz) *nnz = ds->nnz[i];
  return CCO_OK;
}

int cco_dataset_download(const cco_dataset_t *ds, int32_t i, int64_t **row_ptr, int32_t **col_idx) {
  if (!ds || !row_ptr || !col_idx || i < 0 || i >= ds->n_mats) return set_error(CCO_E_INVALID_ARG, "bad argument");
  if (!ds->whole) return set_error(CCO_E_UNSUPPORTED, "this dataset holds one rank's block of users only");
  cco_ctx *c = ds->ctx;
  CK(cudaSetDevice(c->device));
  int64_t *rp = (int64_t *)malloc(sizeof(int64_t) * ((size_t)ds->n_users + 1));
  int32_t *ci = (int32_t *)malloc(sizeof(int32_t) * (size_t)std::max<long long>(ds->nnz[i], 1));
  if (!rp || !ci) return set_error(CCO_E_OOM, "malloc failed");
  CK(cudaStreamSynchronize(c->copy_stream));
  CK(cudaMemcpyAsync(rp, ds->rp_alloc[i], sizeof(int64_t) * ((size_t)ds->n_users + 1), cudaMemcpyDeviceToHost, c->stream));
  if (ds->nnz[i] > 0)
    CK(cudaMemcpyAsync(ci, ds->col_alloc[i], sizeof(int32_t) * (size_t)ds->nnz[i], cudaMemcpyDeviceToHost, c->stream));
  CK(cudaStreamSynchronize(c->stream));
  *row_ptr = rp;
  *col_idx = ci;
  return CCO_OK;
}

struct IngestSource {
  int n_types = 0;
  long long n_users_raw = 0;
  std::vector<long long> n_events;
  std::vector<int32_t> n_items_raw;
  bool keep_item_space = false;
  std::function<int(int, long long *, int32_t *)> fill;
};

static cco_dataset *ingest_dataset_new(cco_ctx *c, int n_types) {
  cco_dataset *d = new cco_dataset();
  d->ctx = c;
  d->n_mats = n_types;
  d->rp.assign(n_types, nullptr);
  d->col.assign(n_types, nullptr);
  d->rp_alloc.assign(n_types, nullptr);
  d->col_alloc.assign(n_types, nullptr);
  d->q_lo.assign(n_types, 0);
  d->q_hi.assign(n_types, 0);
  d->n_cols.assign(n_types, 0);
  d->nnz.assign(n_types, 0);
  d->ready.assign(n_types, nullptr);
  d->validated = true;
  d->whole = true;
  return d;
}

static int ingest_csr(cco_ctx *c, Arena &ar, cco_dataset *d, int t, long long ne, uint32_t n_users, unsigned long long *k0,
                      unsigned long long *k1, unsigned long long kept) {
  cudaStream_t s = c->stream;
  void *p = nullptr;
  cudaError_t e = cudaMallocAsync(&p, sizeof(int64_t) * ((size_t)n_users + 1), s);
  if (e != cudaSuccess) return set_error(CCO_E_OOM, "cudaMallocAsync row_ptr: %s", cudaGetErrorString(e));
  d->rp[t] = (long long *)p;
  d->rp_alloc[t] = p;
  e = cudaMallocAsync(&p, sizeof(int32_t) * (size_t)std::max<unsigned long long>(kept, 4), s);
  if (e != cudaSuccess) return set_error(CCO_E_OOM, "cudaMallocAsync col_idx: %s", cudaGetErrorString(e));
  d->col[t] = (int32_t *)p;
  d->col_alloc[t] = p;
  CK(cudaEventCreateWithFlags(&d->ready[t], cudaEventDisableTiming));
  long long n_unique = 0;
  if (kept > 0)
    CKR(keys_to_csr(c, ar, k0, k1, ne, 64, (long long)kept, n_users, d->col[t], d->rp[t], &n_unique));
  else
    CK(cudaMemsetAsync(d->rp[t], 0, sizeof(int64_t) * ((size_t)n_users + 1), s));
  d->nnz[t] = n_unique;
  CK(cudaEventRecord(d->ready[t], s));
  return CCO_OK;
}

static int ingest_blocks(cco_ctx *c, cco_dataset *d, uint32_t n_users) {
  const int n_types = d->n_mats;
  long long u_lo, u_hi;
  user_block(n_users, c->world, c->rank, &u_lo, &u_hi);
  d->row_base = u_lo;
  d->n_local = u_hi - u_lo;
  for (int t = 0; t < n_types; ++t) {
    CKR(mail_fetch(c, &d->q_lo[t], d->rp[t] + u_lo, 8));
    CKR(mail_fetch(c, &d->q_hi[t], d->rp[t] + u_hi, 8));
  }
  CKR(mail_wait(c));
  for (int t = 0; t < n_types; ++t) d->rp[t] += u_lo;
  return CCO_OK;
}

static int ingest_core(cco_ctx *c, const IngestSource &src, int32_t min_events_per_user, int32_t *user_map,
                       int32_t *const *item_maps, cco_dataset **out) {
  const int n_types = src.n_types;
  const long long n_users_raw = src.n_users_raw;
  *out = nullptr;
  CK(cudaSetDevice(c->device));
  cudaStream_t s = c->stream;
  mail_reset(c);
  Arena ar(s);
  cco_dataset *d = ingest_dataset_new(c, n_types);
  struct G {
    cco_dataset *d;
    bool ok = false;
    ~G() {
      if (!ok) dataset_release(d);
    }
  } g{d};
  const long long nu = std::max<long long>(n_users_raw, 1);
  int32_t *cnt, *d_user_map;
  uint32_t *uflag, *upos;
  CKR(ar.alloc(&cnt, nu));
  CKR(ar.alloc(&uflag, nu + 1));
  CKR(ar.alloc(&upos, nu + 1));
  CKR(ar.alloc(&d_user_map, nu));
  uint32_t n_users = 0;
  for (int t = 0; t < n_types; ++t) {
    const long long ne = src.n_events[t], ni = std::max<int32_t>(src.n_items_raw[t], 1);
    long long *d_user;
    int32_t *d_item;
    CKR(ar.alloc(&d_user, std::max<long long>(ne, 1)));
    CKR(ar.alloc(&d_item, std::max<long long>(ne, 1)));
    if (ne > 0) CKR(src.fill(t, d_user, d_item));
    if (t == 0) {
      CK(cudaMemsetAsync(cnt, 0, sizeof(int32_t) * (size_t)nu, s));
      CK(cudaMemsetAsync(uflag, 0, sizeof(uint32_t) * ((size_t)nu + 1), s));
      if (ne > 0) k_ingest_count_users<<<grid_for(ne, 256, c->sm_count), 256, 0, s>>>(ne, d_user, cnt);
      const int32_t need = min_events_per_user > 1 ? min_events_per_user : 1;
      if (n_users_raw > 0)
        k_ingest_user_flags<<<grid_for(n_users_raw, 256, c->sm_count), 256, 0, s>>>(n_users_raw, cnt, need, uflag);
      CKR(exclusive_sum(c, ar, uflag, upos, nu + 1));
      if (n_users_raw > 0)
        k_ingest_make_map<<<grid_for(n_users_raw, 256, c->sm_count), 256, 0, s>>>(n_users_raw, uflag, upos, d_user_map);
      c->launches += 3;
      CKR(mail_fetch(c, &n_users, upos + n_users_raw, 4));
      if (n_users_raw > 0 && user_map)
        CK(cudaMemcpyAsync(user_map, d_user_map, sizeof(int32_t) * (size_t)n_users_raw, cudaMemcpyDeviceToHost, s));
      CKR(mail_wait(c));
      d->n_users = n_users;
    }
    uint32_t *iflag, *ipos;
    int32_t *d_item_map;
    CKR(ar.alloc(&iflag, ni + 1));
    CKR(ar.alloc(&ipos, ni + 1));
    CKR(ar.alloc(&d_item_map, ni));
    if (src.keep_item_space) {
      CK(cudaMemsetAsync(iflag + ni, 0, 4, s));
      k_fill_u32<<<grid_for(ni, 256, c->sm_count), 256, 0, s>>>(ni, 1u, iflag);
    } else {
      CK(cudaMemsetAsync(iflag, 0, sizeof(uint32_t) * ((size_t)ni + 1), s));
      if (ne > 0) k_ingest_item_flags<<<grid_for(ne, 256, c->sm_count), 256, 0, s>>>(ne, d_user, d_item, d_user_map, iflag);
    }
    CKR(exclusive_sum(c, ar, iflag, ipos, ni + 1));
    k_ingest_make_map<<<grid_for(ni, 256, c->sm_count), 256, 0, s>>>(src.n_items_raw[t], iflag, ipos, d_item_map);
    uint32_t n_items = 0;
    CKR(mail_fetch(c, &n_items, ipos + src.n_items_raw[t], 4));
    if (src.n_items_raw[t] > 0 && item_maps && item_maps[t])
      CK(cudaMemcpyAsync(item_maps[t], d_item_map, sizeof(int32_t) * (size_t)src.n_items_raw[t], cudaMemcpyDeviceToHost, s));
    unsigned long long *k0, *k1, *d_kept;
    CKR(ar.alloc(&k0, std::max<long long>(ne, 1)));
    CKR(ar.alloc(&k1, std::max<long long>(ne, 1)));
    CKR(ar.alloc(&d_kept, 1));
    CK(cudaMemsetAsync(d_kept, 0, 8, s));
    if (ne > 0) k_ingest_keys<<<grid_for(ne, 256, c->sm_count), 256, 0, s>>>(ne, d_user, d_item, d_user_map, d_item_map, k0, d_kept);
    c->launches += 3;
    unsigned long long kept = 0;
    CKR(mail_fetch(c, &kept, d_kept, 8));
    CKR(mail_wait(c));
    ar.release(d_user);
    ar.release(d_item);
    d->n_cols[t] = n_items;
    CKR(ingest_csr(c, ar, d, t, ne, n_users, k0, k1, kept));
    ar.release(k0);
    ar.release(k1);
    ar.release(iflag);
    ar.release(ipos);
    ar.release(d_item_map);
  }
  CKR(ingest_blocks(c, d, n_users));
  CK(cudaStreamSynchronize(s));
  CK(cudaGetLastError());
  g.ok = true;
  *out = d;
  return CCO_OK;
}

int cco_ingest(cco_ctx_t *c, int32_t n_types, const cco_events_t *ev, int64_t n_users_raw, int32_t min_events_per_user,
               int32_t *user_map, int32_t *const *item_maps, cco_dataset_t **out) {
  if (!c || !ev || !user_map || !item_maps || !out || n_types < 1) return set_error(CCO_E_INVALID_ARG, "bad argument");
  if (n_users_raw < 0 || n_users_raw >= 0x7fffffffLL) return set_error(CCO_E_INVALID_ARG, "n_users_raw out of range");
  IngestSource src;
  src.n_types = n_types;
  src.n_users_raw = n_users_raw;
  for (int t = 0; t < n_types; ++t) {
    if (ev[t].n_events < 0 || ev[t].n_events >= 0xffffffffLL || ev[t].n_items_raw < 0)
      return set_error(CCO_E_INVALID_ARG, "type %d: bad event count / item space", t);
    if (ev[t].n_events > 0 && (!ev[t].user || !ev[t].item)) return set_error(CCO_E_INVALID_ARG, "type %d: null event arrays", t);
    if (!item_maps[t] && ev[t].n_items_raw > 0) return set_error(CCO_E_INVALID_ARG, "type %d: null item_map", t);
    for (int64_t i = 0; i < ev[t].n_events; ++i)
      if (ev[t].user[i] < 0 || ev[t].user[i] >= n_users_raw || ev[t].item[i] < 0 || ev[t].item[i] >= ev[t].n_items_raw)
        return set_error(CCO_E_INVALID_ARG, "type %d: user or item id out of range at event %lld", t, (long long)i);
    src.n_events.push_back(ev[t].n_events);
    src.n_items_raw.push_back(ev[t].n_items_raw);
  }
  cudaStream_t s = c->stream;
  src.fill = [&](int t, long long *d_user, int32_t *d_item) -> int {
    CK(cudaMemcpyAsync(d_user, ev[t].user, sizeof(int64_t) * (size_t)ev[t].n_events, cudaMemcpyHostToDevice, s));
    CK(cudaMemcpyAsync(d_item, ev[t].item, sizeof(int32_t) * (size_t)ev[t].n_events, cudaMemcpyHostToDevice, s));
    return CCO_OK;
  };
  return ingest_core(c, src, min_events_per_user, user_map, item_maps, out);
}

int cco_synth_ingest(cco_ctx_t *c, int32_t n_types, const cco_synth_type_t *types, int64_t n_users_raw, const double *user_cdf,
                     const int32_t *user_perm, int32_t min_events_per_user, int32_t keep_item_space, cco_dataset_t **out) {
  if (!c || !types || !out || n_types < 1 || !user_cdf || !user_perm) return set_error(CCO_E_INVALID_ARG, "bad argument");
  if (n_users_raw < 1 || n_users_raw >= 0x7fffffffLL) return set_error(CCO_E_INVALID_ARG, "n_users_raw out of range");
  IngestSource src;
  src.n_types = n_types;
  src.n_users_raw = n_users_raw;
  src.keep_item_space = keep_item_space != 0;
  for (int t = 0; t < n_types; ++t) {
    if (types[t].n_events < 0 || types[t].n_events >= 0xffffffffLL || types[t].n_items < 1 || !types[t].item_cdf || !types[t].item_perm)
      return set_error(CCO_E_INVALID_ARG, "type %d: bad generator spec", t);
    src.n_events.push_back(types[t].n_events);
    src.n_items_raw.push_back(types[t].n_items);
  }
  CK(cudaSetDevice(c->device));
  cudaStream_t s = c->stream;
  double *d_ucdf = nullptr, *d_icdf = nullptr;
  int32_t *d_uperm = nullptr, *d_iperm = nullptr;
  int32_t max_items = 1;
  for (int t = 0; t < n_types; ++t) max_items = std::max(max_items, types[t].n_items);
  auto drop = [&]() {
    for (void *p : {(void *)d_ucdf, (void *)d_icdf, (void *)d_uperm, (void *)d_iperm})
      if (p) cudaFreeAsync(p, s);
  };
  auto up = [&]() -> int {
    CK(cudaMallocAsync((void **)&d_ucdf, sizeof(double) * (size_t)n_users_raw, s));
    CK(cudaMallocAsync((void **)&d_uperm, sizeof(int32_t) * (size_t)n_users_raw, s));
    CK(cudaMallocAsync((void **)&d_icdf, sizeof(double) * (size_t)max_items, s));
    CK(cudaMallocAsync((void **)&d_iperm, sizeof(int32_t) * (size_t)max_items, s));
    CK(cudaMemcpyAsync(d_ucdf, user_cdf, sizeof(double) * (size_t)n_users_raw, cudaMemcpyHostToDevice, s));
    CK(cudaMemcpyAsync(d_uperm, user_perm, sizeof(int32_t) * (size_t)n_users_raw, cudaMemcpyHostToDevice, s));
    return CCO_OK;
  };
  int rc = up();
  if (rc != CCO_OK) { drop(); return rc; }
  src.fill = [&](int t, long long *d_user, int32_t *d_item) -> int {
    CK(cudaMemcpyAsync(d_icdf, types[t].item_cdf, sizeof(double) * (size_t)types[t].n_items, cudaMemcpyHostToDevice, s));
    CK(cudaMemcpyAsync(d_iperm, types[t].item_perm, sizeof(int32_t) * (size_t)types[t].n_items, cudaMemcpyHostToDevice, s));
    k_synth_events<<<grid_for(types[t].n_events, 256, c->sm_count), 256, 0, s>>>(types[t].n_events, types[t].seed, d_ucdf, d_uperm,
                                                                                (int32_t)n_users_raw, d_icdf, d_iperm, types[t].n_items,
                                                                                d_user, d_item);
    c->launches++;
    CK(cudaGetLastError());
    return CCO_OK;
  };
// ... 4468 lines not shown
  *first_member_line = qf->first_member.data();
  return CCO_OK;
}

int cco_query_file_queries(cco_ctx_t *ctx, const cco_query_file_t *qf, const cco_event_log_t *lg, const char *index_body, int64_t index_len,
                           int64_t n_templates, const cco_mixed_query_t *templates, char **out_body, int64_t *out_len, int64_t **out_offsets,
                           int64_t *out_n) {
  if (!ctx || !qf || !out_body || !out_len || !out_offsets || !out_n || index_len < 0 || (index_len > 0 && !index_body) ||
      (n_templates > 0 && !templates))
    return set_error(CCO_E_INVALID_ARG, "null argument or negative length");
  if (qf->ctx != ctx) return set_error(CCO_E_INVALID_ARG, "the query file was read on another context");
  if (lg && lg->ctx != ctx) return set_error(CCO_E_INVALID_ARG, "the log was read on another context");
  if (lg) CKR(log_state(lg, true));
  if (index_len > 0 && index_body[index_len - 1] != '\n') return set_error(CCO_E_INVALID_ARG, "the body does not end in a newline");
  const long long T = (long long)qf->first_line.size();
  if (n_templates != T) return set_error(CCO_E_INVALID_ARG, "%lld templates given, the file has %lld", (long long)n_templates, T);
  static const int64_t zero[1] = {0};
  std::vector<const cco_mixed_query_t *> tq;
  long long user_line = -1, item_line = -1;
  for (long long t = 0; t < T; ++t) {
    const cco_mixed_query_t *q = &templates[t];
    const long long fu = qf->first_member[3 * t], fi = qf->first_member[3 * t + 1];
    const int st = mq_check_host(q, 0, fu >= 0 ? zero : nullptr, nullptr, fi >= 0 ? zero : nullptr, nullptr, nullptr, 0, nullptr, nullptr);
    if (st != CCO_OK) return set_error(st, "line %lld: %s", (long long)qf->first_line[t], std::string(cco_last_error()).c_str());
    if (q->n_blacklist_items != 0) return set_error(CCO_E_INVALID_ARG, "template %lld: blacklistItems are the lines' own", t);
    if (q->n_model_names != templates[0].n_model_names || q->max_query_events != templates[0].max_query_events)
      return set_error(CCO_E_INVALID_ARG, "template %lld: the model names and max_query_events are the algorithm's, the same in every template", t);
    for (int k = 0; k < q->n_model_names; ++k)
      if (strcmp(q->model_names[k], templates[0].model_names[k]) != 0)
        return set_error(CCO_E_INVALID_ARG, "template %lld: the model names are the algorithm's, the same in every template", t);
    if (fu >= 0 && (user_line < 0 || fu < user_line)) user_line = fu;
    if (fi >= 0 && (item_line < 0 || fi < item_line)) item_line = fi;
    tq.push_back(q);
  }
  if (user_line >= 0 && !lg)
    return set_error(CCO_E_INVALID_ARG, "line %lld: a row has a user: its history needs a log (cco_event_log_begin_ex, CCO_LOG_KEEP_HISTORY)", user_line);
  if (user_line >= 0 && !lg->history)
    return set_error(CCO_E_INVALID_ARG, "line %lld: the log was read without history retention (cco_event_log_begin_ex, CCO_LOG_KEEP_HISTORY)", user_line);
  if (item_line >= 0 && !index_body) return set_error(CCO_E_INVALID_ARG, "line %lld: a row has an item: its similar items need an index body", item_line);
  return query_file_queries(ctx, qf, lg, index_body, index_len, tq, out_body, out_len, out_offsets, out_n);
}

int cco_query_file_free(cco_query_file_t *qf) {
  if (!qf) return CCO_OK;
  cudaSetDevice(qf->ctx->device);
  for (void *p : qf->dev) cudaFreeAsync(p, qf->ctx->stream);
  cudaStreamSynchronize(qf->ctx->stream);
  delete qf;
  return CCO_OK;
}

int cco_event_log_free(cco_event_log_t *lg) {
  event_log_release(lg);
  return CCO_OK;
}

int cco_pop_model(cco_ctx_t *ctx, int32_t mode, int64_t n_events, const int32_t *item, const int64_t *time_ms, int32_t n_items,
                  int64_t start_ms, int64_t end_ms, double *score, unsigned char *present) {
  if (!ctx || n_events < 0 || n_items < 0 || (n_events > 0 && (!item || !time_ms)) || (n_items > 0 && (!score || !present)))
    return set_error(CCO_E_INVALID_ARG, "bad argument");
  if (mode < CCO_POP_POPULAR || mode > CCO_POP_HOT) return set_error(CCO_E_INVALID_ARG, "mode must be CCO_POP_POPULAR, _TRENDING or _HOT");
  if (end_ms < start_ms) return set_error(CCO_E_INVALID_ARG, "end before start (Joda Interval would throw)");
  if (n_items == 0) return CCO_OK;
  cco_ctx *c = ctx->members.empty() ? ctx : ctx->members[0];
  CK(cudaSetDevice(c->device));
  cudaStream_t s = c->stream;
  Arena ar(s);
  NvtxRange nvtx("cco:pop_model");
  const PopArgs a = pop_args(mode, start_ms, end_ms, n_items);
  int32_t *d_item, *d_counts;
  long long *d_t;
  unsigned long long *d_tot;
  double *d_score;
  unsigned char *d_present;
  CKR(ar.alloc(&d_item, std::max<long long>(n_events, 1)));
  CKR(ar.alloc(&d_t, std::max<long long>(n_events, 1)));
  CKR(ar.alloc(&d_counts, (size_t)a.n_buckets * n_items));
  CKR(ar.alloc(&d_tot, 4));
  CKR(ar.alloc(&d_score, n_items));
  CKR(ar.alloc(&d_present, n_items));
  CK(cudaMemsetAsync(d_counts, 0, sizeof(int32_t) * (size_t)a.n_buckets * n_items, s));
  CK(cudaMemsetAsync(d_tot, 0, 32, s));
  if (n_events > 0) {
    CK(cudaMemcpyAsync(d_item, item, sizeof(int32_t) * (size_t)n_events, cudaMemcpyHostToDevice, s));
    CK(cudaMemcpyAsync(d_t, time_ms, sizeof(int64_t) * (size_t)n_events, cudaMemcpyHostToDevice, s));
    k_pop_count<<<grid_for(n_events, 256, c->sm_count), 256, 0, s>>>(n_events, d_item, d_t, a, d_counts, d_tot);
    c->launches++;
  }
  k_pop_score<double><<<grid_for(n_items, 256, c->sm_count), 256, 0, s>>>(a, mode, d_counts, d_tot, d_score, d_present);
  c->launches++;
  CK(cudaMemcpyAsync(score, d_score, sizeof(double) * (size_t)n_items, cudaMemcpyDeviceToHost, s));
  CK(cudaMemcpyAsync(present, d_present, (size_t)n_items, cudaMemcpyDeviceToHost, s));
  CK(cudaStreamSynchronize(s));
  CK(cudaGetLastError());
  return CCO_OK;
}

void cco_free(void *p) { free(p); }

int cco_debug_llr(cco_ctx_t *c, int64_t n, const int64_t *k11, const int64_t *k12, const int64_t *k21, const int64_t *k22,
                  uint32_t flags, double *out) {
  if (!c || n < 0 || (n > 0 && (!k11 || !k12 || !k21 || !k22 || !out))) return set_error(CCO_E_INVALID_ARG, "bad argument");
  if (n == 0) return CCO_OK;
  for (int64_t i = 0; i < n; ++i)
    if (k11[i] < 0 || k12[i] < 0 || k21[i] < 0 || k22[i] < 0)
      return set_error(CCO_E_INVALID_ARG, "negative count at %lld (Preconditions.checkArgument in LogLikelihood)", (long long)i);
  CK(cudaSetDevice(c->device));
  Arena ar(c->stream);
  long long *d[4];
  double *dout;
  const int64_t *h[4] = {k11, k12, k21, k22};
  for (int j = 0; j < 4; ++j) {
    CKR(ar.alloc(&d[j], n));
    CK(cudaMemcpyAsync(d[j], h[j], sizeof(int64_t) * (size_t)n, cudaMemcpyHostToDevice, c->stream));
  }
  CKR(ar.alloc(&dout, n));
  k_debug_llr<<<(unsigned)((n + 255) / 256), 256, 0, c->stream>>>(n, d[0], d[1], d[2], d[3], flags, dout);
  CK(cudaMemcpyAsync(out, dout, sizeof(double) * (size_t)n, cudaMemcpyDeviceToHost, c->stream));
  CK(cudaStreamSynchronize(c->stream));
  CK(cudaGetLastError());
  return CCO_OK;
}

int cco_debug_rank_text(cco_ctx_t *c, int64_t n, const int64_t *v, int32_t scale, int64_t *offsets, char *bytes) {
  if (!c || n < 0 || !offsets || (n > 0 && (!v || !bytes))) return set_error(CCO_E_INVALID_ARG, "bad argument");
  if (scale != 0 && scale != 15) return set_error(CCO_E_INVALID_ARG, "scale %d is neither 0 nor 15", scale);
  for (int64_t i = 0; i < n; ++i)
    if (scale == 0 ? (v[i] <= -(1LL << 53) || v[i] >= (1LL << 53)) : (v[i] < 0 || v[i] >= 1000000000000000LL))
      return set_error(CCO_E_INVALID_ARG, "value %lld at %lld is outside the range of scale %d", (long long)v[i], (long long)i, scale);
  offsets[0] = 0;
  if (n == 0) return CCO_OK;
  CK(cudaSetDevice(c->device));
  cudaStream_t s = c->stream;
  Arena ar(s);
  long long *d_v;
  unsigned char *d_slot;
  int32_t *d_len;
  CKR(ar.alloc(&d_v, n));
  CKR(ar.alloc(&d_slot, 32 * n));
  CKR(ar.alloc(&d_len, n));
  CK(cudaMemcpyAsync(d_v, v, sizeof(int64_t) * (size_t)n, cudaMemcpyHostToDevice, s));
  k_debug_rank_text<<<grid_for(n, 256, c->sm_count), 256, 0, s>>>(n, d_v, scale, d_slot, d_len);
  std::vector<unsigned char> slot((size_t)32 * n);
  std::vector<int32_t> len((size_t)n);
  CK(cudaMemcpyAsync(slot.data(), d_slot, slot.size(), cudaMemcpyDeviceToHost, s));
  CK(cudaMemcpyAsync(len.data(), d_len, sizeof(int32_t) * (size_t)n, cudaMemcpyDeviceToHost, s));
  CK(cudaStreamSynchronize(s));
  CK(cudaGetLastError());
  for (int64_t i = 0; i < n; ++i) {
    if (len[i] < 1 || len[i] > 32) return set_error(CCO_E_CUDA, "text %lld has length %d", (long long)i, len[i]);
    memcpy(bytes + offsets[i], slot.data() + 32 * (size_t)i, (size_t)len[i]);
    offsets[i + 1] = offsets[i] + len[i];
  }
  return CCO_OK;
}

int cco_debug_downsample(cco_ctx_t *c, const cco_csr_t *m, int32_t max_interactions, int32_t seed, uint32_t flags,
                         int64_t **row_ptr, int32_t **col_idx, int32_t *raw_col_counts, int32_t *new_col_counts) {
  if (!c || !m || !row_ptr || !col_idx) return set_error(CCO_E_INVALID_ARG, "null argument");
  if (c->world != 1 || !c->members.empty()) return set_error(CCO_E_UNSUPPORTED, "debug entries need a single-GPU context");
  cco_indicator_params_t prm = {max_interactions, 1, 0, 0.0};
  CKR(validate_host(1, m, &prm));
  CK(cudaSetDevice(c->device));
  mail_reset(c);
  c->ev_timing_used = c->ev_plain_used = 0;
  cco_dataset *ds = nullptr;
  CKR(dataset_upload(c, 1, m, flags, &ds));
  struct DG { cco_dataset *d; ~DG() { dataset_release(d); } } dg{ds};
  Arena ar(c->stream);
  Prepared p;
  CKR(prepare(c, ar, ds, &prm, seed, flags, &p));
  const DevMat &dm = p.dm[0];
  std::vector<uint32_t> rp32((size_t)m->n_rows + 1);
  CK(cudaMemcpyAsync(rp32.data(), dm.rp, sizeof(uint32_t) * rp32.size(), cudaMemcpyDeviceToHost, c->stream));
  if (raw_col_counts && m->n_cols > 0)
    CK(cudaMemcpyAsync(raw_col_counts, p.raw_counts, sizeof(int32_t) * (size_t)m->n_cols, cudaMemcpyDeviceToHost, c->stream));
  if (new_col_counts && m->n_cols > 0)
    CK(cudaMemcpyAsync(new_col_counts, dm.marg, sizeof(int32_t) * (size_t)m->n_cols, cudaMemcpyDeviceToHost, c->stream));
  CK(cudaStreamSynchronize(c->stream));
  CK(cudaGetLastError());
  size_t nnz = rp32[m->n_rows];
  int64_t *rp = (int64_t *)malloc(sizeof(int64_t) * rp32.size());
  int32_t *ci = (int32_t *)calloc(std::max<size_t>(nnz, 1), sizeof(int32_t));
  if (!rp || !ci) return set_error(CCO_E_OOM, "malloc failed");
  for (size_t i = 0; i < rp32.size(); ++i) rp[i] = rp32[i];
  const size_t n_copy = std::min<size_t>(nnz, (size_t)ds->nnz[0]);
  if (n_copy) CK(cudaMemcpy(ci, dm.col, sizeof(int32_t) * n_copy, cudaMemcpyDeviceToHost));
  *row_ptr = rp;
  *col_idx = ci;
  return CCO_OK;
}

int cco_debug_downsample_block(cco_ctx_t *c, const cco_csr_t *m, int64_t row_lo, int64_t row_hi, const int32_t *raw_col_counts,
                               int32_t max_interactions, int32_t seed, uint32_t flags, int64_t *kept_per_row, int32_t **col_idx,
                               int32_t *new_col_counts) {
  if (!c || !m || !col_idx || (m->n_rows > 0 && !kept_per_row) || (m->n_cols > 0 && (!raw_col_counts || !new_col_counts)))
    return set_error(CCO_E_INVALID_ARG, "null argument");
  if (c->world != 1 || !c->members.empty()) return set_error(CCO_E_UNSUPPORTED, "debug entries need a single-GPU context");
  cco_indicator_params_t prm = {max_interactions, 1, 0, 0.0};
  CKR(validate_host(1, m, &prm));
  if (row_lo < 0 || row_hi < row_lo || row_hi > m->n_rows)
    return set_error(CCO_E_INVALID_ARG, "rows [%lld, %lld) outside [0, %lld)", (long long)row_lo, (long long)row_hi, (long long)m->n_rows);
  CK(cudaSetDevice(c->device));
  mail_reset(c);
  cudaStream_t s = c->stream;
  cco_dataset *ds = nullptr;
  CKR(dataset_upload(c, 1, m, flags, &ds));
  struct DG { cco_dataset *d; ~DG() { dataset_release(d); } } dg{ds};
  Arena ar(s);
  const long long U = ds->n_users;
  const int32_t width = std::max<int32_t>(m->n_cols, 1);
  long long q[2] = {0, 0};
  CK(cudaMemcpyAsync(&q[0], ds->rp[0] + row_lo, sizeof(long long), cudaMemcpyDeviceToHost, s));
  CK(cudaMemcpyAsync(&q[1], ds->rp[0] + row_hi, sizeof(long long), cudaMemcpyDeviceToHost, s));
  CK(cudaStreamSynchronize(s));
  DevRaw blk;
  blk.n_rows = row_hi - row_lo;
  blk.row_base = row_lo;
  blk.n_cols = m->n_cols;
  blk.q_base = q[0];
  blk.nnz = q[1] - q[0];
  blk.rp = ds->rp[0] + row_lo;
  blk.col = ds->col[0];
  int32_t *counts, *marg, *dst;
  uint32_t *kept;
  CKR(ar.alloc(&counts, width));
  CKR(ar.alloc(&marg, width));
  CKR(ar.alloc(&kept, U + 1));
  CKR(ar.alloc(&dst, std::max<long long>(blk.nnz, 1)));
  if (m->n_cols > 0) CK(cudaMemcpyAsync(counts, raw_col_counts, sizeof(int32_t) * (size_t)m->n_cols, cudaMemcpyHostToDevice, s));
  CK(cudaMemsetAsync(marg, 0, sizeof(int32_t) * (size_t)width, s));
  CK(cudaMemsetAsync(kept, 0, sizeof(uint32_t) * ((size_t)U + 1), s));
  SampleScratch sc;
  CKR(sample_scratch(c, ar, blk, counts, max_interactions, &sc));
  launch_count(c, blk, sc, max_interactions, seed, flags, nullptr, kept, marg);
  CKR(launch_write(c, ar, blk, sc, dst));
  std::vector<uint32_t> hk((size_t)U + 1);
  CK(cudaMemcpyAsync(hk.data(), kept, sizeof(uint32_t) * hk.size(), cudaMemcpyDeviceToHost, s));
  if (m->n_cols > 0) CK(cudaMemcpyAsync(new_col_counts, marg, sizeof(int32_t) * (size_t)m->n_cols, cudaMemcpyDeviceToHost, s));
  CK(cudaStreamSynchronize(s));
  CK(cudaGetLastError());
  size_t n_kept = 0;
  for (long long r = 0; r < U; ++r) {
    kept_per_row[r] = hk[r];
    if (r >= row_lo && r < row_hi) n_kept += hk[r];
  }
  int32_t *ci = (int32_t *)calloc(std::max<size_t>(n_kept, 1), sizeof(int32_t));
  if (!ci) return set_error(CCO_E_OOM, "malloc failed");
  const size_t n_copy = std::min<size_t>(n_kept, (size_t)blk.nnz);
  if (n_copy) {
    cudaError_t e = cudaMemcpy(ci, dst, sizeof(int32_t) * n_copy, cudaMemcpyDeviceToHost);
    if (e != cudaSuccess) {
      free(ci);
      return set_error(CCO_E_CUDA, "cudaMemcpy: %s", cudaGetErrorString(e));
    }
  }
  *col_idx = ci;
  return CCO_OK;
}

int cco_debug_key_range_cap(cco_ctx_t *c, int32_t max_keys) {
  if (!c || max_keys < 0) return set_error(CCO_E_INVALID_ARG, "null context or negative cap");
  c->key_range_cap = max_keys;
  for (cco_ctx *m : c->members) m->key_range_cap = max_keys;
  return CCO_OK;
}

int cco_debug_intern_hash_bits(cco_ctx_t *c, int32_t bits) {
  if (!c || bits < 0 || bits > 64) return set_error(CCO_E_INVALID_ARG, "null context or hash bits %d not in [0, 64]", bits);
  c->intern_mask = bits == 64 ? ~0ULL : (1ULL << bits) - 1;
  return CCO_OK;
}

int cco_debug_cooccurrence(cco_ctx_t *c, const cco_csr_t *a, const cco_csr_t *b, int64_t **row_ptr, int32_t **col_idx,
                           int32_t **count) {
  if (!c || !a || !b || !row_ptr || !col_idx || !count) return set_error(CCO_E_INVALID_ARG, "null argument");
  if (c->world != 1 || !c->members.empty()) return set_error(CCO_E_UNSUPPORTED, "debug entries need a single-GPU context");
  cco_csr_t two[2] = {*a, *b};
  cco_indicator_params_t prm[2] = {{0x7fffffff, 1, 0, 0.0}, {0x7fffffff, 1, 0, 0.0}};
  CKR(validate_host(2, two, prm));
  CK(cudaSetDevice(c->device));
  mail_reset(c);
  c->ev_timing_used = c->ev_plain_used = 0;
  cco_dataset *ds = nullptr;
  CKR(dataset_upload(c, 2, two, 0, &ds));
  struct DG { cco_dataset *d; ~DG() { dataset_release(d); } } dg{ds};
  Arena ar(c->stream);
  struct CopyJoin {
    cco_ctx *c;
    ~CopyJoin() { cudaStreamSynchronize(c->copy_stream); }
  } copy_join{c};
  Prepared prep;
  CKR(prepare(c, ar, ds, prm, 0, 0, &prep));
  const int32_t n_items_a = prep.dm[0].n_cols;
  ResultMat rm;
  IndicatorOut io;
  IndicatorState ist;
  struct EG { IndicatorState &x; ~EG() { if (x.packed) cudaEventDestroy(x.packed); } } eg{ist};
  cco_indicator_params_t p1 = {0x7fffffff, 1, 0, 0.0};
  auto put = [&]() {
    for (void *p : {(void *)rm.row_ptr, (void *)rm.col, (void *)rm.llr, (void *)rm.cnt})
      if (p) c->pinned_put(p);
  };
  int rc = enqueue_indicator(c, ar, prep.at_ptr, prep.at_users, n_items_a, prep.dm[0].marg, prep.max_marg[0], prep.max_marg[1], prep.dm[1],
                             a->n_rows, false, p1, 0, true, nullptr, nullptr, nullptr, &ist);
  if (rc == CCO_OK) rc = finish_indicator(c, &ist, 0, 0, &rm, &io);
  cudaStreamSynchronize(c->copy_stream);
  if (rc != CCO_OK) {
    put();
    return rc;
  }
  size_t nnz = (size_t)rm.row_ptr[n_items_a];
  int64_t *rp = (int64_t *)malloc(sizeof(int64_t) * ((size_t)n_items_a + 1));
  int32_t *ci = (int32_t *)malloc(sizeof(int32_t) * std::max<size_t>(nnz, 1));
  int32_t *cn = (int32_t *)malloc(sizeof(int32_t) * std::max<size_t>(nnz, 1));
  if (!rp || !ci || !cn) {
    put();
    return set_error(CCO_E_OOM, "malloc failed");
  }
  memcpy(rp, rm.row_ptr, sizeof(int64_t) * ((size_t)n_items_a + 1));
  std::vector<std::pair<int32_t, int32_t>> tmp;
  for (int32_t r = 0; r < n_items_a; ++r) {
    size_t lo = (size_t)rp[r], hi = (size_t)rp[r + 1];
    tmp.resize(hi - lo);
    for (size_t q = lo; q < hi; ++q) tmp[q - lo] = {rm.col[q], rm.cnt[q]};
    std::sort(tmp.begin(), tmp.end());
    for (size_t q = lo; q < hi; ++q) {
      ci[q] = tmp[q - lo].first;
      cn[q] = tmp[q - lo].second;
    }
  }
  put();
  *row_ptr = rp;
  *col_idx = ci;
  *count = cn;
  return CCO_OK;
}

extern "C++" {
namespace cco {

struct ReaderLatch {
  bool failed = false, finished = false;
  std::string msg;
  int code = CCO_OK;
  int fail(int st) {
    failed = true;
    code = st;
    msg = cco_last_error();
    return st;
  }
  int state(const char *finished_msg) const {
    if (failed) return set_error(code == CCO_OK ? CCO_E_INVALID_ARG : code, "%s", msg.c_str());
    if (finished) return set_error(CCO_E_INVALID_ARG, "%s", finished_msg);
    return CCO_OK;
  }
};

struct BodyStage {
  char *pinned[2] = {};
  size_t pinned_cap[2] = {};
  unsigned char *dev[2] = {};
  size_t dev_cap[2] = {};
  cudaEvent_t copied[2] = {};

  int init() {
    for (cudaEvent_t &e : copied)
      if (cudaEventCreateWithFlags(&e, cudaEventDisableTiming) != cudaSuccess) return set_error(CCO_E_CUDA, "cudaEventCreate failed");
    return CCO_OK;
  }
  int put(cco_ctx *c, int slot, const char *bytes, long long len, const char *what, const char *copy_of) {
    const size_t padded = (size_t)((len + 63) / 64 * 64) + 64;
    size_t free_b = 0, total_b = 0;
    CK(cudaMemGetInfo(&free_b, &total_b));
    if (padded > total_b / 4) return set_error(CCO_E_UNSUPPORTED, "%s: at most a quarter of the device's memory", what);
    if (pinned_cap[slot] < padded) {
      if (pinned[slot]) cudaFreeHost(pinned[slot]);
      pinned[slot] = nullptr;
      pinned_cap[slot] = 0;
      if (cudaHostAlloc((void **)&pinned[slot], padded, cudaHostAllocPortable) != cudaSuccess)
        return set_error(CCO_E_OOM, "cudaHostAlloc(%zu) failed", padded);
      pinned_cap[slot] = padded;
    }
    if (dev_cap[slot] < padded) {
      if (dev[slot]) cudaFree(dev[slot]);
      dev[slot] = nullptr;
      dev_cap[slot] = 0;
      if (cudaMalloc((void **)&dev[slot], padded) != cudaSuccess) return set_error(CCO_E_UNSUPPORTED, "%s does not fit the device", what);
      dev_cap[slot] = padded;
    }
    if (len > 0) memcpy(pinned[slot], bytes, (size_t)len);
    memset(pinned[slot] + len, ' ', padded - (size_t)len);
    if (cudaMemcpyAsync(dev[slot], pinned[slot], padded, cudaMemcpyHostToDevice, c->copy_stream) != cudaSuccess ||
        cudaEventRecord(copied[slot], c->copy_stream) != cudaSuccess)
      return set_error(CCO_E_CUDA, "the copy of %s failed", copy_of);
    return CCO_OK;
  }
  int wait(cudaStream_t s, int slot) const {
    CK(cudaStreamWaitEvent(s, copied[slot], 0));
    return CCO_OK;
  }
  const char *host(int slot) const { return pinned[slot]; }
  void release(cco_ctx *c) {
    cudaStreamSynchronize(c->copy_stream);
    for (int i = 0; i < 2; ++i) {
      if (pinned[i]) cudaFreeHost(pinned[i]);
      if (dev[i]) cudaFree(dev[i]);
      if (copied[i]) cudaEventDestroy(copied[i]);
    }
  }
};

static const char *sr_message(int code) {
  switch (code) {
    case kSrSyntax: return "malformed JSON";
    case kSrString: return "a string holds a bad escape or a raw byte < 0x20";
    case kSrUnbalanced: return "unbalanced or mismatched brackets";
    case kSrNoResponses: return "the top level is not an object with one \"responses\" array";
    case kSrElement: return "a responses element is not an object";
    case kSrStatus: return "status is not a 32-bit integer";
    case kSrHitsNotArray: return "hits.hits is not an array";
    case kSrHitNotObject: return "a hits.hits element is not an object";
    case kSrNoId: return "the hit has no string _id";
    case kSrRepeated: return "a repeated _id or _score";
    case kSrNoScore: return "_score is missing, null or not a number";
    case kSrBadRank: return "a rank is not a number";
    case kSrLine: return "the query line is not one JSON object";
    case kSrWithRanks: return "the query line's withRanks is not true, false or null";
    case kSrLineRepeated: return "the query line repeats withRanks";
    case kSrLineDeep: return "the query line nests deeper than 64 levels";
    case kSrOpenString: return "a string is not closed";
    case kSrNotObject: return "the top level is not an object";
    case kSrEsError: return "Elasticsearch returned an error";
    case kSrRepeatedId: return "a repeated _id";
    case kIpTimedOut: return "the search timed out (timed_out is true)";
    case kIpShards: return "_shards.failed is not 0";
    case kIpHitsNotArray: return "hits.hits is neither an array nor absent";
    case kIpNoSource: return "the hit has no _source";
    case kIpSourceNotObject: return "_source is not an object";
    case kIwNoItems: return "the response has no \"items\" array";
    case kIwItemNotObject: return "an items element is not an object";
    case kIwNotIndex: return "the item is not {\"index\":{...}}";
    case kIwNoId: return "the item has no string _id";
    case kIwIdMismatch: return "the item's _id is not the document's _id";
    case kIwNoStatus: return "the item has no status";
    case kIwRepeatedStatus: return "a repeated status";
    case kIwBadStatus: return "the status is not a 32-bit integer";
  }
  return "malformed response";
}

struct SrIndex {
  long long *pos = nullptr;
  unsigned char *dep = nullptr;
  long long m = 0;
};
static int sr_index(cco_ctx *c, Arena &ar, const unsigned char *body, long long len, int max_depth, SrIndex *ix, unsigned long long *bad) {
  cudaStream_t s = c->stream;
  const long long NW = (len + 63) / 64, n_chunks = (NW + kSrChunkWords - 1) / kSrChunkWords;
  unsigned long long *err;
  SrFun *fun, *pre;
  long long *cnt, *coff;
  CKR(ar.alloc(&err, 1));
  CKR(ar.alloc(&fun, n_chunks + 1));
  CKR(ar.alloc(&pre, n_chunks + 1));
  CKR(ar.alloc(&cnt, n_chunks + 1));
  CKR(ar.alloc(&coff, n_chunks + 1));
  CK(cudaMemsetAsync(err, 0xff, 8, s));
  CK(cudaMemsetAsync(cnt + n_chunks, 0, 8, s));
  SrFun fin = sr_identity();
  if (n_chunks > 0) {
    const int grid = grid_for(n_chunks * 32, 256, c->sm_count);
    k_sr_chunk<<<grid, 256, 0, s>>>(NW, (const uint4 *)body, fun);
    k_sr_scan<<<1, kSrScanThreads, 0, s>>>(n_chunks, fun, pre);
    k_sr_index<false><<<grid, 256, 0, s>>>(NW, (const uint4 *)body, pre, max_depth, cnt, nullptr, nullptr, nullptr, err);
    c->launches += 3;
    CKR(mail_fetch(c, &fin, pre + n_chunks - 1, sizeof(SrFun)));
  }
  CKR(exclusive_sum(c, ar, cnt, coff, n_chunks + 1));
  ix->m = 0;
  *bad = ~0ULL;
  CKR(mail_fetch(c, &ix->m, coff + n_chunks, 8));
  CKR(mail_fetch(c, bad, err, 8));
  CKR(mail_wait(c));
  if (*bad == ~0ULL && (fin.f[0] >> 1)) *bad = (unsigned long long)len << 8 | kSrOpenString;
  if (*bad == ~0ULL && fin.d[0] != 0) *bad = (unsigned long long)len << 8 | kSrUnbalanced;
  if (*bad == ~0ULL) {
    CKR(ar.alloc(&ix->pos, ix->m + 1));
    CKR(ar.alloc(&ix->dep, ix->m + 1));
    if (ix->m > 0) {
      k_sr_index<true><<<grid_for(n_chunks * 32, 256, c->sm_count), 256, 0, s>>>(NW, (const uint4 *)body, pre, max_depth, nullptr, coff, ix->pos,
                                                                                  ix->dep, err);
      c->launches++;
    }
  }
  for (void *p : {(void *)err, (void *)fun, (void *)pre, (void *)cnt, (void *)coff}) ar.release(p);
  return CCO_OK;
}

template <typename T>
static int pinned_give(cco_ctx *c, T **out, const void *src, size_t n) {
  *out = (T *)c->pinned_get(std::max<size_t>(n, 1), false);
  if (!*out) return set_error(CCO_E_OOM, "pinned host allocation failed");
  if (src && n) memcpy(*out, src, n);
  return CCO_OK;
}

static std::string sr_unescape(const char *p, long long n) {
  std::string o;
  auto hex4 = [](const char *q) { return (unsigned)strtoul(std::string(q, 4).c_str(), nullptr, 16); };
  for (long long i = 0; i < n;) {
    if (p[i] != '\\') {
      o += p[i++];
      continue;
    }
    const char x = p[i + 1];
    if (x != 'u') {
      o += x == 'b' ? '\b' : x == 'f' ? '\f' : x == 'n' ? '\n' : x == 'r' ? '\r' : x == 't' ? '\t' : x;
      i += 2;
      continue;
    }
    unsigned cp = hex4(p + i + 2);
    i += 6;
    if (cp >= 0xd800 && cp < 0xdc00 && i + 6 <= n && p[i] == '\\' && p[i + 1] == 'u') {
      const unsigned lo = hex4(p + i + 2);
      if (lo >= 0xdc00 && lo < 0xe000) {
        cp = 0x10000 + ((cp - 0xd800) << 10) + (lo - 0xdc00);
        i += 6;
      }
    }
    if (cp < 0x80) {
      o += (char)cp;
    } else if (cp < 0x800) {
      o += (char)(0xc0 | cp >> 6);
      o += (char)(0x80 | (cp & 0x3f));
    } else if (cp < 0x10000) {
      o += (char)(0xe0 | cp >> 12);
      o += (char)(0x80 | (cp >> 6 & 0x3f));
      o += (char)(0x80 | (cp & 0x3f));
    } else {
      o += (char)(0xf0 | cp >> 18);
      o += (char)(0x80 | (cp >> 12 & 0x3f));
      o += (char)(0x80 | (cp >> 6 & 0x3f));
      o += (char)(0x80 | (cp & 0x3f));
    }
  }
  return o;
}

}
}

struct cco_search_results {
  cco_ctx *ctx = nullptr;
  int n_rank = 0;
  uint32_t flags = 0;
  std::string names, qnames;
  int name_off[9] = {}, qname_off[9] = {};
  BodyStage stage;
  long long n_bodies = 0;
  bool pending = false;
  long long p_len = 0, p_rec = 0;
  std::vector<uint8_t> p_ranks;
  bool p_has_lines = false;
  std::vector<int64_t> p_loff;
  std::string p_lines;
  ReaderLatch latch;
  std::vector<int64_t> hit_off{0}, total, id_off{0}, text_off{0};
  std::vector<int32_t> status;
  std::vector<double> score, ranks;
  std::string id_bytes, text;
  long long n_exact = 0;
};

extern "C++" {
namespace cco {

static int sr_count_check(long long n, const char *what) {
  if (n >= (1LL << 31)) return set_error(CCO_E_UNSUPPORTED, "%lld %s in one body: at most 2^31 - 1", n, what);
  return CCO_OK;
}
static int sr_exact_value(const char *t, long long n, SrNum *o) {
  std::string s(t, (size_t)n);
  const double v = strtod(s.c_str(), nullptr);
  if (std::isinf(v)) return 1;
  SrNum r = {v, 0ULL, 0, 0, s[0] == '-', 0};
  if (v != 0) {
    char buf[40];
    const std::to_chars_result tc = std::to_chars(buf, buf + sizeof buf - 1, std::fabs(v), std::chars_format::scientific);
    *tc.ptr = 0;
    const char *e = strchr(buf, 'e');
    unsigned long long dig = 0;
    int nd = 0;
    for (const char *q = buf; q < e; ++q)
      if (*q != '.') {
        dig = dig * 10 + (unsigned)(*q - '0');
        ++nd;
      }
    int e10 = atoi(e + 1) - (nd - 1);
    while (dig % 10 == 0) {
      dig /= 10;
      ++e10;
      --nd;
    }
    r.dig = dig;
    r.e10 = e10;
    r.nd = nd;
  }
// ... 1087 lines not shown
```

Measured before the change: 4.473 billion.

## Split indicator enqueue into plan/order/schedule/run stages overlapped across streams

Breaks the indicator pipeline into separate plan, column-order, schedule and run stages. The column-order and schedule work for later matrices is issued on a side stream while earlier matrices run, and the packing/compaction tail moves to a new pack stream. The host now waits only on an early mailbox group holding the max marginals and validity checks, which are computed earlier in downsampling, instead of the full mailbox. Per-kernel occupancy and smem attribute queries are cached. This adds cross-stream event dependencies and moves some arena frees to a different stream, which raises the risk of ordering bugs.

```diff
diff --git a/universal_recommender_b200/csrc/cco_api.cu b/universal_recommender_b200/csrc/cco_api.cu
--- a/universal_recommender_b200/csrc/cco_api.cu
+++ b/universal_recommender_b200/csrc/cco_api.cu
@@ -140,6 +140,7 @@
   cudaEvent_t copy_ev[2] = {};
   cudaStream_t bin_stream[8] = {};
   cudaStream_t sched_stream = nullptr;
+  cudaStream_t pack_stream = nullptr;
   cudaEvent_t bin_ev[9] = {};
   std::vector<PinnedBuf> pinned;
   std::mutex mu;
@@ -299,10 +300,15 @@
       }
     return 0;
   }
-  void release(void *p) {
+  void release_all() {
+    for (void *p : ptrs) cudaFreeAsync(p, s);
+    ptrs.clear();
+    sizes.clear();
+  }
+  void release(void *p, cudaStream_t on = nullptr) {
     for (size_t i = 0; i < ptrs.size(); ++i)
       if (ptrs[i] == p) {
-        cudaFreeAsync(p, s);
+        cudaFreeAsync(p, on ? on : s);
         ptrs.erase(ptrs.begin() + i);
         sizes.erase(sizes.begin() + i);
         return;
@@ -337,22 +343,22 @@
 }
 
 constexpr size_t kMailBytes = 1 << 16;
-static int mail_fetch(cco_ctx *c, void *dst_host, const void *src_dev, size_t n) {
+static int mail_fetch(cco_ctx *c, void *dst_host, const void *src_dev, size_t n, cudaStream_t on = nullptr) {
   size_t off = (c->mail_used + 7) & ~(size_t)7;
   if (off + n > kMailBytes) return set_error(CCO_E_CUDA, "internal: mailbox overflow");
-  k_mail_bytes<<<1, 128, 0, c->stream>>>(c->mail_d + off, (const unsigned char *)src_dev, (int)n);
+  k_mail_bytes<<<1, 128, 0, on ? on : c->stream>>>(c->mail_d + off, (const unsigned char *)src_dev, (int)n);
   c->mail_pending.push_back({dst_host, off, n, c->mail_group});
   c->mail_used = off + n;
   return CCO_OK;
 }
-static int mail_close(cco_ctx *c, int *group) {
+static int mail_close(cco_ctx *c, int *group, cudaStream_t on = nullptr) {
   const int g = c->mail_group;
   while ((int)c->mail_ev.size() <= g) {
     cudaEvent_t e;
     CK(cudaEventCreateWithFlags(&e, cudaEventDisableTiming));
     c->mail_ev.push_back(e);
   }
-  CK(cudaEventRecord(c->mail_ev[g], c->stream));
+  CK(cudaEventRecord(c->mail_ev[g], on ? on : c->stream));
   c->mail_group = g + 1;
   if (group) *group = g;
   return CCO_OK;
@@ -616,10 +622,11 @@
   return CCO_OK;
 }
 
-static int downsample_all(cco_ctx *c, Arena &ar, const std::vector<DevRaw> &raw, const int *d_check , long long U,
+static int downsample_all(cco_ctx *c, Arena &ar, const std::vector<DevRaw> &raw, int *d_check , long long U,
                           const int32_t *raw_counts, int32_t *marg_all, const std::vector<long long> &col_off,
                           const cco_indicator_params_t *params, int32_t seed, uint32_t flags, std::vector<DevMat> &dm,
-                          const cudaEvent_t *stage_ev ) {
+                          const cudaEvent_t *stage_ev , int32_t *d_max, int32_t *h_max, int *h_check, cudaEvent_t marg_ready,
+                          int *early_group) {
   cudaStream_t s = c->stream;
   const int W = c->world, r = c->rank, n_mats = (int)raw.size();
   const long long S = (U + W - 1) / W;
@@ -649,6 +656,16 @@
     if (col_off[n_mats] > 0)
       CKR(nccl_check(g_nccl.AllReduce(marg_all, marg_all, (size_t)col_off[n_mats], kNcclInt32, kNcclSum, c->comm, s), "ncclAllReduce(marginals)"));
   }
+  for (int i = 0; i < n_mats; ++i)
+    if (dm[i].n_cols > 0) {
+      k_max_i32<<<grid_for(dm[i].n_cols, 256, c->sm_count, 2), 256, 0, s>>>(dm[i].n_cols, dm[i].marg, d_max + i);
+      c->launches++;
+    }
+  CK(cudaEventRecord(marg_ready, s));
+  CKR(mail_fetch(c, h_max, d_max, 4 * (size_t)n_mats));
+  CKR(mail_fetch(c, h_check, d_check, sizeof(int) * 2 * (size_t)n_mats));
+  *early_group = -1;
+  if (W == 1) CKR(mail_close(c, early_group));
   std::vector<uint32_t> edge((size_t)n_mats * (W + 1), 0);
   for (int i = 0; i < n_mats; ++i) {
     CKR(exclusive_sum(c, ar, kept[i], dm[i].rp, U + 1));
@@ -719,6 +736,30 @@
   return p;
 }
 
+struct RowsOcc { int device; const void *fn; size_t smem; int occ; };
+static std::mutex g_rows_occ_mu;
+static std::vector<RowsOcc> g_rows_occ;
+static std::vector<RowsOcc> g_rows_smem_limit;
+static int rows_occupancy(cco_ctx *c, const void *fn, int cta, size_t smem, int *occ) {
+  std::lock_guard<std::mutex> lk(g_rows_occ_mu);
+  for (const RowsOcc &e : g_rows_occ)
+    if (e.device == c->device && e.fn == fn && e.smem == smem) {
+      *occ = e.occ;
+      return CCO_OK;
+    }
+  RowsOcc *lim = nullptr;
+  for (RowsOcc &e : g_rows_smem_limit)
+    if (e.device == c->device && e.fn == fn) lim = &e;
+  if (!lim || lim->smem < smem) {
+    CK(cudaFuncSetAttribute(fn, cudaFuncAttributeMaxDynamicSharedMemorySize, (int)smem));
+    if (lim) lim->smem = smem;
+    else g_rows_smem_limit.push_back({c->device, fn, smem, 0});
+  }
+  CK(cudaOccupancyMaxActiveBlocksPerMultiprocessor(occ, fn, cta, smem));
+  g_rows_occ.push_back({c->device, fn, smem, *occ});
+  return CCO_OK;
+}
+
 template <int GROUP>
 static int launch_rows_t(cco_ctx *c, const RowArgs &a, BinCfg &cfg, cudaStream_t st) {
   constexpr int CTA = GROUP == 32 ? 64 : GROUP;
@@ -728,8 +769,7 @@
     if (cfg.bitmap) kern = k_rows<GROUP, false, true>;
   if constexpr (GROUP == 32)
     if (cfg.sorted) kern = k_rows<32, false, false, true>;
-  CK(cudaFuncSetAttribute(kern, cudaFuncAttributeMaxDynamicSharedMemorySize, (int)cfg.smem));
-  CK(cudaOccupancyMaxActiveBlocksPerMultiprocessor(&occ, kern, CTA, cfg.smem));
+  CKR(rows_occupancy(c, (const void *)kern, CTA, cfg.smem, &occ));
   kern<<<c->sm_count * std::max(occ, 1) * 4, CTA, cfg.smem, st>>>(a);
   cfg.ctas_per_sm = occ;
   c->launches++;
@@ -927,127 +967,167 @@
   int32_t n_items_a = 0, n_cols_b = 0;
   int n_ranges = 1;
   bool emit_all = false;
+  bool beside = false, split = false;
+  cudaStream_t ss = nullptr;
+  cudaEvent_t scheduled = nullptr;
+  int32_t max_marg_a = 0, max_marg_b = 0;
+  long long n_users = 0;
+  int k_eff = 1, count_bits = 0, cb_bits = 1;
+  long long k11_max = 0;
+  int32_t stride = 1;
+  size_t cells = 1, sort_tb = 0, order_tb = 0;
+  uint32_t *row_work = nullptr, *masked = nullptr, *sorted_work = nullptr;
+  unsigned long long *work64 = nullptr;
+  long long *work_prefix = nullptr;
+  int32_t *ids = nullptr, *rows_sorted = nullptr, *d_pb = nullptr;
+  int32_t *key_of_col = nullptr, *first_key_of_cb = nullptr;
+  const int32_t *marg_key = nullptr, *col_of_key = nullptr;
+  int32_t *o_len = nullptr;
+  unsigned long long *d_distinct = nullptr;
+  int *d_err = nullptr;
+  BinPlan bins;
 };
 
-static int enqueue_indicator(cco_ctx *c, Arena &ar, const uint32_t *at_ptr, const int32_t *at_users, int32_t n_items_a,
-                             const int32_t *marg_a, int32_t max_marg_a, int32_t max_marg_b, const DevMat &B, long long n_users,
-                             bool self, const cco_indicator_params_t &prm, uint32_t flags, bool emit_all, cudaEvent_t inputs_ready,
-                             cudaEvent_t ev_begin, cudaEvent_t ev_end, IndicatorState *st) {
+static int indicator_plan(cco_ctx *c, const Arena &ar, int32_t n_items_a, int32_t max_marg_a, int32_t max_marg_b, int32_t n_cols_b,
+                          long long n_users, const cco_indicator_params_t &prm, uint32_t flags, bool emit_all, bool side,
+                          IndicatorState *st) {
   cudaStream_t s = c->stream;
-  const int32_t n_cols_b = B.n_cols;
-  const int rank = c->rank, world = c->world;
   st->n_items_a = n_items_a;
   st->n_cols_b = n_cols_b;
   st->emit_all = emit_all;
-  uint32_t *row_work, *masked, *sorted_work;
-  unsigned long long *work64;
-  long long *work_prefix;
-  int32_t *ids, *rows_sorted, *d_pb = nullptr;
-  size_t sort_tb = 0, order_tb = 0;
+  st->max_marg_a = max_marg_a;
+  st->max_marg_b = max_marg_b;
+  st->n_users = n_users;
+  st->n_ranges = 1;
   if (n_items_a > 0)
-    CK(cub::DeviceRadixSort::SortPairsDescending(nullptr, sort_tb, (const uint32_t *)nullptr, (uint32_t *)nullptr, (const int32_t *)nullptr,
+    CK(cub::DeviceRadixSort::SortPairsDescending(nullptr, st->sort_tb, (const uint32_t *)nullptr, (uint32_t *)nullptr, (const int32_t *)nullptr,
                                                  (int32_t *)nullptr, n_items_a, 0, 32, s));
-  int cb_bits = 1;
-  while ((1LL << cb_bits) <= (long long)max_marg_b) ++cb_bits;
+  st->cb_bits = 1;
+  while ((1LL << st->cb_bits) <= (long long)max_marg_b) ++st->cb_bits;
   cub::DoubleBuffer<uint32_t> order_cb(nullptr, nullptr);
   cub::DoubleBuffer<int32_t> order_id(nullptr, nullptr);
-  if (n_cols_b > 0) CK(cub::DeviceRadixSort::SortPairs(nullptr, order_tb, order_cb, order_id, n_cols_b, 0, cb_bits, s));
-  const bool beside = inputs_ready && ar.c && ((size_t)n_items_a + 1) * 8 <= Arena::kSlabMax && sort_tb <= Arena::kSlabMax &&
-                      (size_t)n_cols_b * 4 <= Arena::kSlabMax && order_tb <= Arena::kSlabMax &&
-                      ((size_t)max_marg_b + 2) * 4 <= Arena::kSlabMax;
-  cudaStream_t ss = beside ? c->sched_stream : s;
-  if (beside) CK(cudaStreamWaitEvent(ss, inputs_ready, 0));
-  CKR(ar.alloc(&row_work, n_items_a + 1));
-  CKR(ar.alloc(&masked, n_items_a + 1));
-  CKR(ar.alloc(&work64, n_items_a + 1));
-  CKR(ar.alloc(&work_prefix, n_items_a + 1));
-  CKR(ar.alloc(&ids, n_items_a + 1));
-  CKR(ar.alloc(&sorted_work, n_items_a + 1));
-  CKR(ar.alloc(&rows_sorted, n_items_a + 1));
-  CK(cudaMemsetAsync(work64 + n_items_a, 0, 8, ss));
-  k_row_work<<<grid_for((long long)n_items_a * kSG, 256, c->sm_count), 256, 0, ss>>>(n_items_a, at_ptr, at_users, B.rp,
-                                                                                  row_work, work64, ids, nullptr);
-  c->launches++;
-  CKR(exclusive_sum(c, ar, (const long long *)work64, work_prefix, (long long)n_items_a + 1, ss));
-  if (world > 1) {
-    CKR(ar.alloc(&d_pb, world + 1));
-    k_partition_rows<<<1, ((world + 1 + 31) / 32) * 32, 0, ss>>>(work_prefix, n_items_a, world, d_pb);
-    c->launches++;
-  }
-  k_mask_work<<<grid_for(n_items_a, 256, c->sm_count), 256, 0, ss>>>(n_items_a, row_work, d_pb, rank, masked);
-  c->launches++;
-  if (n_items_a > 0) {
-    void *tmp;
-    CKR(ar.alloc((char **)&tmp, sort_tb));
-    CK(cub::DeviceRadixSort::SortPairsDescending(tmp, sort_tb, masked, sorted_work, ids, rows_sorted, n_items_a, 0, 32, ss));
-    ar.release(tmp);
-  }
-  const int k_eff = emit_all ? 1 : prm.top_k;
-  int key_bits, count_bits;
-  const long long k11_max = std::min<long long>(max_marg_a, max_marg_b);
-  const bool fits = packed_bits(n_cols_b, k11_max, &key_bits, &count_bits);
-  const bool split = n_cols_b > 0 && (c->key_range_cap > 0 || (!fits && (flags & CCO_FLAG_KEY_RANGES)));
-  if (!fits && !split)
+  if (n_cols_b > 0) CK(cub::DeviceRadixSort::SortPairs(nullptr, st->order_tb, order_cb, order_id, n_cols_b, 0, st->cb_bits, s));
+  st->k_eff = emit_all ? 1 : prm.top_k;
+  int key_bits;
+  st->k11_max = std::min<long long>(max_marg_a, max_marg_b);
+  const bool fits = packed_bits(n_cols_b, st->k11_max, &key_bits, &st->count_bits);
+  st->split = n_cols_b > 0 && (c->key_range_cap > 0 || (!fits && (flags & CCO_FLAG_KEY_RANGES)));
+  if (!fits && !st->split)
     return set_error(CCO_E_UNSUPPORTED,
                      "co-occurrence counts up to %lld over %d columns do not fit the packed 32-bit accumulator word "
                      "(key %d bits + count %d bits): lower maxItemsPerUser/maxEventsPerEventType for this event type, "
                      "or train it in key ranges with CCO_FLAG_KEY_RANGES (\"Limits\" in include/cco_b200.h)",
-                     k11_max, n_cols_b, key_bits, count_bits);
-  st->n_ranges = 1;
-  BinPlan bins;
-  if (!split)
-    CKR(plan_bins(c, ar, n_items_a, n_cols_b, count_bits, max_marg_a, max_marg_b, n_users, k_eff, emit_all, sorted_work, ss, &bins));
-  int32_t *key_of_col, *first_key_of_cb, *order_id0, *order_id1;
+                     st->k11_max, n_cols_b, key_bits, st->count_bits);
+  st->beside = side && ar.c && !st->split && ((size_t)n_items_a + 1) * 8 <= Arena::kSlabMax && st->sort_tb <= Arena::kSlabMax &&
+               (size_t)n_cols_b * 4 <= Arena::kSlabMax && st->order_tb <= Arena::kSlabMax &&
+               ((size_t)max_marg_b + 2) * 4 <= Arena::kSlabMax;
+  st->ss = st->beside ? c->sched_stream : s;
+  st->stride = std::max<int32_t>(emit_all ? n_cols_b : std::min<int32_t>(prm.top_k, n_cols_b), 1);
+  st->cells = (size_t)std::max(n_items_a, 1) * st->stride;
+  return CCO_OK;
+}
+
+static int indicator_order(cco_ctx *c, Arena &ar, const DevMat &B, cudaEvent_t marg_ready, IndicatorState *st) {
+  cudaStream_t ss = st->ss;
+  if (st->beside) CK(cudaStreamWaitEvent(ss, marg_ready, 0));
+  const int32_t n_cols_b = st->n_cols_b, n_order = std::max<int32_t>(n_cols_b, 1);
+  int32_t *order_id0, *order_id1;
   uint32_t *order_cb0, *order_cb1;
-  const int32_t n_order = std::max<int32_t>(n_cols_b, 1);
-  CKR(ar.alloc(&key_of_col, n_order));
-  CKR(ar.alloc(&first_key_of_cb, (size_t)max_marg_b + 2));
+  CKR(ar.alloc(&st->key_of_col, n_order));
+  CKR(ar.alloc(&st->first_key_of_cb, (size_t)st->max_marg_b + 2));
   CKR(ar.alloc(&order_cb0, n_order));
   CKR(ar.alloc(&order_cb1, n_order));
   CKR(ar.alloc(&order_id0, n_order));
   CKR(ar.alloc(&order_id1, n_order));
-  order_cb = cub::DoubleBuffer<uint32_t>(order_cb0, order_cb1);
-  order_id = cub::DoubleBuffer<int32_t>(order_id0, order_id1);
+  cub::DoubleBuffer<uint32_t> order_cb(order_cb0, order_cb1);
+  cub::DoubleBuffer<int32_t> order_id(order_id0, order_id1);
   if (n_cols_b > 0) {
     k_col_order_init<<<grid_for(n_cols_b, 256, c->sm_count, 4), 256, 0, ss>>>(n_cols_b, B.marg, order_cb0, order_id0);
     void *tmp;
-    CKR(ar.alloc((char **)&tmp, order_tb));
-    CK(cub::DeviceRadixSort::SortPairs(tmp, order_tb, order_cb, order_id, n_cols_b, 0, cb_bits, ss));
+    CKR(ar.alloc((char **)&tmp, st->order_tb));
+    CK(cub::DeviceRadixSort::SortPairs(tmp, st->order_tb, order_cb, order_id, n_cols_b, 0, st->cb_bits, ss));
     ar.release(tmp);
-    k_col_order<<<grid_for(n_cols_b, 256, c->sm_count, 4), 256, 0, ss>>>(n_cols_b, max_marg_b, order_cb.Current(), order_id.Current(),
-                                                                        key_of_col, first_key_of_cb);
-    k_relabel_cols<<<c->sm_count * 8, 256, 0, ss>>>(B.rp + B.n_rows, key_of_col, B.col);
-    c->launches += 3;
-  }
-  const int32_t *marg_key = reinterpret_cast<const int32_t *>(order_cb.Current()), *col_of_key = order_id.Current();
-  if (beside) {
-    cudaEvent_t scheduled;
-    CKR(pooled_event(c, false, &scheduled));
-    CK(cudaEventRecord(scheduled, ss));
-    CK(cudaStreamWaitEvent(s, scheduled, 0));
-  }
+    k_col_order<<<grid_for(n_cols_b, 256, c->sm_count, 4), 256, 0, ss>>>(n_cols_b, st->max_marg_b, order_cb.Current(), order_id.Current(),
+                                                                        st->key_of_col, st->first_key_of_cb);
+    c->launches += 2;
+  }
+  st->marg_key = reinterpret_cast<const int32_t *>(order_cb.Current());
+  st->col_of_key = order_id.Current();
+  CKR(ar.alloc(&st->o_len, st->n_items_a + 1));
+  CKR(ar.alloc(&st->d_distinct, 2));
+  CKR(ar.alloc(&st->d_err, 1));
+  CK(cudaMemsetAsync(st->o_len, 0, sizeof(int32_t) * ((size_t)st->n_items_a + 1), ss));
+  CK(cudaMemsetAsync(st->d_distinct, 0, 16, ss));
+  CK(cudaMemsetAsync(st->d_err, 0, 4, ss));
+  return CCO_OK;
+}
+
+static int indicator_schedule(cco_ctx *c, Arena &ar, const uint32_t *at_ptr, const int32_t *at_users, const DevMat &B,
+                              cudaEvent_t prep_done, IndicatorState *st) {
+  cudaStream_t ss = st->ss;
+  const int32_t n_items_a = st->n_items_a, n_cols_b = st->n_cols_b;
+  if (st->beside) CK(cudaStreamWaitEvent(ss, prep_done, 0));
+  if (n_cols_b > 0) {
+    k_relabel_cols<<<c->sm_count * 8, 256, 0, ss>>>(B.rp + B.n_rows, st->key_of_col, B.col);
+    c->launches++;
+  }
+  CKR(ar.alloc(&st->row_work, n_items_a + 1));
+  CKR(ar.alloc(&st->masked, n_items_a + 1));
+  CKR(ar.alloc(&st->work64, n_items_a + 1));
+  CKR(ar.alloc(&st->work_prefix, n_items_a + 1));
+  CKR(ar.alloc(&st->ids, n_items_a + 1));
+  CKR(ar.alloc(&st->sorted_work, n_items_a + 1));
+  CKR(ar.alloc(&st->rows_sorted, n_items_a + 1));
+  CK(cudaMemsetAsync(st->work64 + n_items_a, 0, 8, ss));
+  k_row_work<<<grid_for((long long)n_items_a * kSG, 256, c->sm_count), 256, 0, ss>>>(n_items_a, at_ptr, at_users, B.rp, st->row_work,
+                                                                                  st->work64, st->ids, nullptr);
+  c->launches++;
+  CKR(exclusive_sum(c, ar, (const long long *)st->work64, st->work_prefix, (long long)n_items_a + 1, ss));
+  if (c->world > 1) {
+    CKR(ar.alloc(&st->d_pb, c->world + 1));
+    k_partition_rows<<<1, ((c->world + 1 + 31) / 32) * 32, 0, ss>>>(st->work_prefix, n_items_a, c->world, st->d_pb);
+    c->launches++;
+  }
+  k_mask_work<<<grid_for(n_items_a, 256, c->sm_count), 256, 0, ss>>>(n_items_a, st->row_work, st->d_pb, c->rank, st->masked);
+  c->launches++;
+  if (n_items_a > 0) {
+    void *tmp;
+    CKR(ar.alloc((char **)&tmp, st->sort_tb));
+    CK(cub::DeviceRadixSort::SortPairsDescending(tmp, st->sort_tb, st->masked, st->sorted_work, st->ids, st->rows_sorted, n_items_a, 0, 32, ss));
+    ar.release(tmp);
+  }
+  if (!st->split)
+    CKR(plan_bins(c, ar, n_items_a, n_cols_b, st->count_bits, st->max_marg_a, st->max_marg_b, st->n_users, st->k_eff, st->emit_all,
+                  st->sorted_work, ss, &st->bins));
+  if (st->beside) {
+    CKR(pooled_event(c, false, &st->scheduled));
+    CK(cudaEventRecord(st->scheduled, ss));
+  }
+  return CCO_OK;
+}
+
+static int indicator_run(cco_ctx *c, Arena &ar, const uint32_t *at_ptr, const int32_t *at_users, const int32_t *marg_a, const DevMat &B,
+                         bool self, const cco_indicator_params_t &prm, uint32_t flags, cudaEvent_t ev_begin, cudaEvent_t ev_end,
+                         IndicatorState *st) {
+  cudaStream_t s = c->stream;
+  const int32_t n_items_a = st->n_items_a, n_cols_b = st->n_cols_b, max_marg_a = st->max_marg_a, max_marg_b = st->max_marg_b;
+  const long long n_users = st->n_users;
+  const int rank = c->rank, k_eff = st->k_eff;
+  const bool emit_all = st->emit_all;
+  const int32_t stride = st->stride;
+  const size_t cells = st->cells;
+  if (st->beside) CK(cudaStreamWaitEvent(s, st->scheduled, 0));
   ColTerm *col_terms;
   CKR(ar.alloc(&col_terms, std::max<int32_t>(n_cols_b, 1)));
   if (n_cols_b > 0) {
-    k_col_terms<<<grid_for(n_cols_b, 256, c->sm_count, 4), 256, 0, s>>>(n_cols_b, marg_key, col_of_key, n_users, flags, col_terms);
-    c->launches++;
-  }
-  int32_t stride = emit_all ? n_cols_b : std::min<int32_t>(prm.top_k, n_cols_b);
-  if (stride < 1) stride = 1;
-  int32_t *o_col, *o_cnt, *o_len;
+    k_col_terms<<<grid_for(n_cols_b, 256, c->sm_count, 4), 256, 0, s>>>(n_cols_b, st->marg_key, st->col_of_key, n_users, flags, col_terms);
+    c->launches++;
+  }
+  int32_t *o_col, *o_cnt;
   double *o_llr = nullptr;
-  unsigned long long *d_distinct;
-  int *d_err;
-  size_t cells = (size_t)std::max(n_items_a, 1) * stride;
   CKR(ar.alloc(&o_col, cells));
   CKR(ar.alloc(&o_cnt, cells));
   if (!emit_all) CKR(ar.alloc(&o_llr, cells));
-  CKR(ar.alloc(&o_len, n_items_a + 1));
-  CKR(ar.alloc(&d_distinct, 2));
-  CKR(ar.alloc(&d_err, 1));
-  CK(cudaMemsetAsync(o_len, 0, sizeof(int32_t) * ((size_t)n_items_a + 1), s));
-  CK(cudaMemsetAsync(d_distinct, 0, 16, s));
-  CK(cudaMemsetAsync(d_err, 0, 4, s));
   RowArgs a;
   memset(&a, 0, sizeof a);
   a.at_ptr = at_ptr;
@@ -1055,14 +1135,14 @@
   a.b_ptr = B.rp;
   a.b_col = B.col;
   a.marg_a = marg_a;
-  a.marg_b = marg_key;
-  a.key_of_col = key_of_col;
-  a.first_key_of_cb = first_key_of_cb;
+  a.marg_b = st->marg_key;
+  a.key_of_col = st->key_of_col;
+  a.first_key_of_cb = st->first_key_of_cb;
   a.key_shift = key_shift_for(n_cols_b);
   a.max_marg_b = max_marg_b;
   a.col_terms = col_terms;
-  a.rows_sorted = rows_sorted;
-  a.row_work = row_work;
+  a.rows_sorted = st->rows_sorted;
+  a.row_work = st->row_work;
   a.n_cols_b = n_cols_b;
   a.n_users = n_users;
   a.self = self ? 1 : 0;
@@ -1072,26 +1152,26 @@
   a.cut_ok = cut_exact(n_users, max_marg_a, max_marg_b) ? 1 : 0;
   a.llr_eps2 = 2.0 * llr_error_bound(n_users);
   a.flags = flags;
-  a.count_bits = count_bits;
+  a.count_bits = st->count_bits;
   a.out_stride = stride;
   a.out_col = o_col;
   a.out_llr = o_llr;
   a.out_cnt = o_cnt;
-  a.out_len = o_len;
-  a.stat_distinct = d_distinct;
-  a.stat_evaluated = d_distinct + 1;
-  a.err_flag = d_err;
+  a.out_len = st->o_len;
+  a.stat_distinct = st->d_distinct;
+  a.stat_evaluated = st->d_distinct + 1;
+  a.err_flag = st->d_err;
   a.emit_all = emit_all ? 1 : 0;
   a.key_base = 0;
   if (ev_begin) CK(cudaEventRecord(ev_begin, s));
-  if (!split) {
-    if (n_items_a > 0) CKR(launch_bins(c, a, bins, s));
+  if (!st->split) {
+    if (n_items_a > 0) CKR(launch_bins(c, a, st->bins, s));
   } else {
     const int32_t n_fk = max_marg_b + 2;
     int32_t *h_fk = (int32_t *)c->pinned_get(sizeof(int32_t) * ((size_t)n_fk + 1), false);
     if (!h_fk) return set_error(CCO_E_OOM, "pinned host allocation failed");
     struct PutBack { cco_ctx *c; void *p; ~PutBack() { c->pinned_put(p); } } put_back{c, h_fk};
-    CK(cudaMemcpyAsync(h_fk, first_key_of_cb, sizeof(int32_t) * (size_t)n_fk, cudaMemcpyDeviceToHost, s));
+    CK(cudaMemcpyAsync(h_fk, st->first_key_of_cb, sizeof(int32_t) * (size_t)n_fk, cudaMemcpyDeviceToHost, s));
     CK(cudaMemcpyAsync(h_fk + n_fk, B.rp + B.n_rows, sizeof(uint32_t), cudaMemcpyDeviceToHost, s));
     CK(cudaStreamSynchronize(s));
     std::vector<KeyRange> plan;
@@ -1099,7 +1179,7 @@
       return set_error(CCO_E_UNSUPPORTED,
                        "co-occurrence counts up to %lld do not fit the packed 32-bit accumulator word even in a key range of one "
                        "column (at most 2^30 - 1): lower maxItemsPerUser/maxEventsPerEventType for this event type "
-                       "(\"Limits\" in include/cco_b200.h)", k11_max);
+                       "(\"Limits\" in include/cco_b200.h)", st->k11_max);
     const long long nnz_b = (long long)(uint32_t)h_fk[n_fk], U = B.n_rows;
     st->n_ranges = (int)plan.size();
     uint32_t *r_cnt, *r_ptr;
@@ -1113,7 +1193,7 @@
     CKR(ar.alloc(&r_col, std::max<long long>(nnz_b, 1)));
     CKR(ar.alloc(&fk_r, (size_t)max_marg_b + 2));
     CKR(ar.alloc((char **)&scan_tmp, scan_tb));
-    CKR(ar.alloc((char **)&sort_tmp, sort_tb));
+    CKR(ar.alloc((char **)&sort_tmp, st->sort_tb));
     BinPlan bp;
     if (plan.size() > 1) {
       CKR(ar.alloc(&t_col, cells));
@@ -1129,22 +1209,22 @@
       CK(cub::DeviceScan::ExclusiveSum(scan_tmp, scan_tb, r_cnt, r_ptr, U + 1, s));
       k_split_range<true><<<split_grid, 256, 0, s>>>(U, B.rp, B.col, kr.k0, kr.k1, r_ptr, r_col);
       c->launches += 2;
-      k_row_work<<<grid_for((long long)n_items_a * kSG, 256, c->sm_count), 256, 0, s>>>(n_items_a, at_ptr, at_users, r_ptr, row_work,
-                                                                                     work64, ids, nullptr);
-      k_mask_work<<<grid_for(n_items_a, 256, c->sm_count), 256, 0, s>>>(n_items_a, row_work, d_pb, rank, masked);
+      k_row_work<<<grid_for((long long)n_items_a * kSG, 256, c->sm_count), 256, 0, s>>>(n_items_a, at_ptr, at_users, r_ptr, st->row_work,
+                                                                                     st->work64, st->ids, nullptr);
+      k_mask_work<<<grid_for(n_items_a, 256, c->sm_count), 256, 0, s>>>(n_items_a, st->row_work, st->d_pb, rank, st->masked);
       c->launches += 2;
       if (n_items_a > 0)
-        CK(cub::DeviceRadixSort::SortPairsDescending(sort_tmp, sort_tb, masked, sorted_work, ids, rows_sorted, n_items_a, 0, 32, s));
-      k_range_first_keys<<<grid_for((long long)kr.max_marg + 2, 256, c->sm_count), 256, 0, s>>>(kr.max_marg + 2, first_key_of_cb, kr.k0,
+        CK(cub::DeviceRadixSort::SortPairsDescending(sort_tmp, st->sort_tb, st->masked, st->sorted_work, st->ids, st->rows_sorted, n_items_a, 0, 32, s));
+      k_range_first_keys<<<grid_for((long long)kr.max_marg + 2, 256, c->sm_count), 256, 0, s>>>(kr.max_marg + 2, st->first_key_of_cb, kr.k0,
                                                                                              n_r, fk_r);
       c->launches++;
       int kb_r, cbits_r;
       packed_bits(n_r, std::min<long long>(max_marg_a, kr.max_marg), &kb_r, &cbits_r);
-      CKR(plan_bins(c, ar, n_items_a, n_r, cbits_r, max_marg_a, kr.max_marg, n_users, k_eff, emit_all, sorted_work, s, &bp));
+      CKR(plan_bins(c, ar, n_items_a, n_r, cbits_r, max_marg_a, kr.max_marg, n_users, k_eff, emit_all, st->sorted_work, s, &bp));
       RowArgs ar_r = a;
       ar_r.b_ptr = r_ptr;
       ar_r.b_col = r_col;
-      ar_r.marg_b = marg_key + kr.k0;
+      ar_r.marg_b = st->marg_key + kr.k0;
       ar_r.col_terms = col_terms + kr.k0;
       ar_r.first_key_of_cb = fk_r;
       ar_r.key_base = kr.k0;
@@ -1163,36 +1243,43 @@
       if (n_items_a > 0) CKR(launch_bins(c, ar_r, bp, s));
       if (r > 0 && n_items_a > 0) {
         k_merge_range<<<grid_for((long long)n_items_a * 32, 256, c->sm_count), 256, 0, s>>>(n_items_a, stride, k_eff, emit_all ? 1 : 0, o_col,
-                                                                                         o_llr, o_cnt, o_len, t_col, t_llr, t_cnt, t_len);
+                                                                                         o_llr, o_cnt, st->o_len, t_col, t_llr, t_cnt, t_len);
         c->launches++;
       }
     }
   }
   if (ev_end) CK(cudaEventRecord(ev_end, s));
+  cudaStream_t ps = st->beside ? c->pack_stream : s;
   long long *len64, *rec_d;
   CKR(ar.alloc(&len64, n_items_a + 1));
   CKR(ar.alloc(&st->out_ptr, n_items_a + 1));
   CKR(ar.alloc(&rec_d, 8));
-  k_len_to_i64<<<grid_for((long long)n_items_a + 1, 256, c->sm_count), 256, 0, s>>>(n_items_a, o_len, d_pb, rank, len64);
-  c->launches++;
-  CKR(exclusive_sum(c, ar, len64, st->out_ptr, (long long)n_items_a + 1));
   CKR(ar.alloc(&st->p_col, cells));
   if (!(flags & CCO_FLAG_RESULT_NO_COUNT) || emit_all) CKR(ar.alloc(&st->p_cnt, cells));
   if (!emit_all && !(flags & CCO_FLAG_RESULT_NO_LLR)) CKR(ar.alloc(&st->p_llr, cells));
+  if (st->beside) {
+    cudaEvent_t joined;
+    CKR(pooled_event(c, false, &joined));
+    CK(cudaEventRecord(joined, s));
+    CK(cudaStreamWaitEvent(ps, joined, 0));
+  }
+  k_len_to_i64<<<grid_for((long long)n_items_a + 1, 256, c->sm_count), 256, 0, ps>>>(n_items_a, st->o_len, st->d_pb, rank, len64);
+  c->launches++;
+  CKR(exclusive_sum(c, ar, len64, st->out_ptr, (long long)n_items_a + 1, ps));
   if (n_items_a > 0) {
-    k_compact_rows<<<grid_for((long long)n_items_a * 32, 256, c->sm_count), 256, 0, s>>>(n_items_a, stride, st->out_ptr, o_col, o_llr,
-                                                                                      o_cnt, st->p_col, st->p_llr, st->p_cnt);
-    c->launches++;
-  }
-  k_indicator_record<<<1, 32, 0, s>>>(n_items_a, d_pb, rank, st->out_ptr, work_prefix, d_distinct, d_err, rec_d);
+    k_compact_rows<<<grid_for((long long)n_items_a * 32, 256, c->sm_count), 256, 0, ps>>>(n_items_a, stride, st->out_ptr, o_col, o_llr,
+                                                                                       o_cnt, st->p_col, st->p_llr, st->p_cnt);
+    c->launches++;
+  }
+  k_indicator_record<<<1, 32, 0, ps>>>(n_items_a, st->d_pb, rank, st->out_ptr, st->work_prefix, st->d_distinct, st->d_err, rec_d);
   c->launches++;
-  CKR(mail_fetch(c, st->rec, rec_d, sizeof(long long) * 7));
-  CKR(mail_close(c, &st->mail_group));
+  CKR(mail_fetch(c, st->rec, rec_d, sizeof(long long) * 7, ps));
+  CKR(mail_close(c, &st->mail_group, ps));
   if (!st->packed) CK(cudaEventCreateWithFlags(&st->packed, cudaEventDisableTiming));
-  CK(cudaEventRecord(st->packed, s));
+  CK(cudaEventRecord(st->packed, ps));
   CK(cudaGetLastError());
   for (void *p : {(void *)o_col, (void *)o_cnt, (void *)o_llr, (void *)len64})
-    if (p) ar.release(p);
+    if (p) ar.release(p, ps);
   return CCO_OK;
 }
 
@@ -1460,6 +1547,7 @@
   std::vector<int32_t> max_marg;
   std::vector<uint32_t> nnz;
   cudaEvent_t stage[7] = {};
+  cudaEvent_t marg_ready = nullptr;
 };
 static int prepare(cco_ctx *c, Arena &ar, const cco_dataset *ds, const cco_indicator_params_t *params, int32_t seed, uint32_t flags,
                    Prepared *p) {
@@ -1496,15 +1584,21 @@
   CK(mark(1));
   std::vector<DevMat> &dm = p->dm;
   dm.assign(n_mats, DevMat());
-  CKR(downsample_all(c, ar, raw, d_check, n_users, p->raw_counts, marg_all, col_off, params, seed, flags, dm, &p->stage[2]));
+  int32_t *d_max;
+  CKR(ar.alloc(&d_max, n_mats));
+  CK(cudaMemsetAsync(d_max, 0, 4 * (size_t)n_mats, s));
+  CKR(pooled_event(c, false, &p->marg_ready));
+  p->max_marg.assign(n_mats, 0);
+  p->nnz.assign(n_mats, 0);
+  std::vector<int> h_check(2 * n_mats, 0);
+  int early_group = -1;
+  CKR(downsample_all(c, ar, raw, d_check, n_users, p->raw_counts, marg_all, col_off, params, seed, flags, dm, &p->stage[2], d_max,
+                     p->max_marg.data(), h_check.data(), p->marg_ready, &early_group));
   const int32_t n_items_a = dm[0].n_cols;
   uint32_t *cursor;
-  int32_t *d_max;
   CKR(ar.alloc(&p->at_ptr, n_items_a + 1));
   CKR(ar.alloc(&cursor, n_items_a + 1));
-  CKR(ar.alloc(&d_max, n_mats));
   CKR(ar.alloc(&p->at_users, std::max<long long>(ds->nnz[0], 1)));
-  CK(cudaMemsetAsync(d_max, 0, 4 * (size_t)n_mats, s));
   {
     uint32_t *marg_pad;
     CKR(ar.alloc(&marg_pad, n_items_a + 1));
@@ -1517,21 +1611,11 @@
   k_transpose_entries<<<grid_for((ds->nnz[0] + kSampleChunk - 1) / kSampleChunk * 32, 256, c->sm_count), 256, 0, s>>>(n_users, dm[0].rp,
                                                                                                                      dm[0].col, cursor, p->at_users);
   c->launches++;
-  for (int i = 0; i < n_mats; ++i)
-    if (dm[i].n_cols > 0) {
-      k_max_i32<<<grid_for(dm[i].n_cols, 256, c->sm_count, 2), 256, 0, s>>>(dm[i].n_cols, dm[i].marg, d_max + i);
-      c->launches++;
-    }
-  p->max_marg.assign(n_mats, 0);
-  p->nnz.assign(n_mats, 0);
-  std::vector<int> h_check(2 * n_mats, 0);
-  CKR(mail_fetch(c, p->max_marg.data(), d_max, 4 * (size_t)n_mats));
-  CKR(mail_fetch(c, h_check.data(), d_check, sizeof(int) * 2 * (size_t)n_mats));
   for (int i = 0; i < n_mats; ++i) CKR(mail_fetch(c, &p->nnz[i], dm[i].rp + n_users, 4));
   CK(mark(6));
   CK(cudaEventRecord(c->ev[2], s));
   nvtx_pop();
-  CKR(mail_wait(c));
+  if (early_group >= 0) CKR(mail_wait_group(c, early_group));
   for (int i = 0; i < n_mats; ++i)
     if (h_check[2 * i]) return set_error(CCO_E_INVALID_ARG, "matrix %d: row_ptr not monotone or column index out of [0, n_cols)", i);
   return CCO_OK;
@@ -1550,6 +1634,7 @@
     ~CopyJoin() {
       cudaStreamSynchronize(c->copy_stream);
       cudaStreamSynchronize(c->sched_stream);
+      cudaStreamSynchronize(c->pack_stream);
     }
   } copy_join{c};
   cco_result *res = new cco_result();
@@ -1574,23 +1659,36 @@
   for (int i = 0; i < n_mats; ++i) st.nnz_in_total += ds->nnz[i];
   Prepared p;
   CKR(prepare(c, ar, ds, params, seed, flags, &p));
-  for (int i = 0; i < n_mats && i < 16; ++i) st.nnz_downsampled[i] = p.nnz[i];
 
   const int32_t n_items_a = p.dm[0].n_cols;
   std::vector<IndicatorOut> io(n_mats);
   std::vector<cudaEvent_t> ev_rows(2 * n_mats, nullptr);
   for (auto &e : ev_rows) CKR(pooled_event(c, true, &e));
+  for (int i = 0; i < n_mats; ++i)
+    CKR(indicator_plan(c, ar, n_items_a, p.max_marg[0], p.max_marg[i], p.dm[i].n_cols, n_users, params[i], flags, false, true, &ist[i]));
+  for (int i = 0; i < n_mats; ++i)
+    if (ist[i].beside) CKR(indicator_order(c, ar, p.dm[i], p.marg_ready, &ist[i]));
+  if (ist[0].beside) CKR(indicator_schedule(c, ar, p.at_ptr, p.at_users, p.dm[0], c->ev[2], &ist[0]));
   for (int i = 0; i < n_mats; ++i) {
     nvtx_push("cco:indicator");
-    CKR(enqueue_indicator(c, ar, p.at_ptr, p.at_users, n_items_a, p.dm[0].marg, p.max_marg[0], p.max_marg[i], p.dm[i], n_users, i == 0,
-                          params[i], flags, false, c->ev[2], ev_rows[2 * i], ev_rows[2 * i + 1], &ist[i]));
+    if (!ist[i].beside) {
+      CKR(indicator_order(c, ar, p.dm[i], nullptr, &ist[i]));
+      CKR(indicator_schedule(c, ar, p.at_ptr, p.at_users, p.dm[i], nullptr, &ist[i]));
+    }
+    CKR(indicator_run(c, ar, p.at_ptr, p.at_users, p.dm[0].marg, p.dm[i], i == 0, params[i], flags, ev_rows[2 * i], ev_rows[2 * i + 1],
+                      &ist[i]));
+    if (i + 1 < n_mats && ist[i + 1].beside) CKR(indicator_schedule(c, ar, p.at_ptr, p.at_users, p.dm[i + 1], c->ev[2], &ist[i + 1]));
     nvtx_pop();
     if (i > 0) CKR(finish_indicator(c, &ist[i - 1], flags, i - 1, &res->mats[i - 1], &io[i - 1]));
   }
   CKR(finish_indicator(c, &ist[n_mats - 1], flags, n_mats - 1, &res->mats[n_mats - 1], &io[n_mats - 1]));
+  for (int i = 0; i < n_mats && i < 16; ++i) st.nnz_downsampled[i] = p.nnz[i];
   CK(cudaEventRecord(c->copy_ev[1], c->copy_stream));
   CK(cudaStreamWaitEvent(s, c->copy_ev[1], 0));
+  for (auto &x : ist)
+    if (x.beside) CK(cudaStreamWaitEvent(s, x.packed, 0));
   CK(cudaEventRecord(c->ev[3], s));
+  ar.release_all();
   CK(cudaStreamSynchronize(s));
   CK(cudaStreamSynchronize(c->copy_stream));
   for (int i = 0; i < n_mats && i < 16; ++i) {
@@ -1731,6 +1829,7 @@
   int lo_pri = 0, hi_pri = 0;
   CK(cudaDeviceGetStreamPriorityRange(&lo_pri, &hi_pri));
   CK(cudaStreamCreateWithPriority(&c->sched_stream, cudaStreamNonBlocking, hi_pri));
+  CK(cudaStreamCreateWithFlags(&c->pack_stream, cudaStreamNonBlocking));
   for (auto &ev : c->bin_ev) CK(cudaEventCreateWithFlags(&ev, cudaEventDisableTiming));
   CK(cudaHostAlloc((void **)&c->mail_h, kMailBytes, cudaHostAllocMapped | cudaHostAllocPortable));
   CK(cudaHostGetDevicePointer((void **)&c->mail_d, c->mail_h, 0));
@@ -1876,6 +1975,7 @@
   for (auto &st : c->bin_stream)
     if (st) cudaStreamDestroy(st);
   if (c->sched_stream) cudaStreamDestroy(c->sched_stream);
+  if (c->pack_stream) cudaStreamDestroy(c->pack_stream);
   for (auto &ev : c->bin_ev)
     if (ev) cudaEventDestroy(ev);
   if (c->stream) cudaStreamDestroy(c->stream);
@@ -6950,8 +7050,10 @@
     for (void *p : {(void *)rm.row_ptr, (void *)rm.col, (void *)rm.llr, (void *)rm.cnt})
       if (p) c->pinned_put(p);
   };
-  int rc = enqueue_indicator(c, ar, prep.at_ptr, prep.at_users, n_items_a, prep.dm[0].marg, prep.max_marg[0], prep.max_marg[1], prep.dm[1],
-                             a->n_rows, false, p1, 0, true, nullptr, nullptr, nullptr, &ist);
+  int rc = indicator_plan(c, ar, n_items_a, prep.max_marg[0], prep.max_marg[1], prep.dm[1].n_cols, a->n_rows, p1, 0, true, false, &ist);
+  if (rc == CCO_OK) rc = indicator_order(c, ar, prep.dm[1], nullptr, &ist);
+  if (rc == CCO_OK) rc = indicator_schedule(c, ar, prep.at_ptr, prep.at_users, prep.dm[1], nullptr, &ist);
+  if (rc == CCO_OK) rc = indicator_run(c, ar, prep.at_ptr, prep.at_users, prep.dm[0].marg, prep.dm[1], false, p1, 0, nullptr, nullptr, &ist);
   if (rc == CCO_OK) rc = finish_indicator(c, &ist, 0, 0, &rm, &io);
   cudaStreamSynchronize(c->copy_stream);
   if (rc != CCO_OK) {
```

Measured after the change: 4.553 billion (median of 6 runs). +1.8%, better.
